# Siyou-Li/u2Tokenizer

Measured on AMD Instinct MI355X. Metric: CT volumes/sec (256^3 fp16) through u2Tokenizer fwd, higher is better.
Workload: dtype bf16; 1 GPU; BASELINE configs[2]: u2Qwen3-8B-shaped path, 256^3 volume = 8x(32,256,256) fp16, ViT-B 3D x12, SPP, 4-layer rma+diffts+dmtp tokenizer (8 heads, top_k 1024, scales {1,2,4}, 256 queries), text 1024, prompt 1024; hidden_size=4096, batch_per_gpu=1, streams_per_gpu=2, parallelism=replicas x1, tta_side_stream=off in the multi-stream run, on in the one-stream run

## Files before the change

### u2tokenizer_amd/checkpoint.py

```python
from __future__ import annotations

import os
from typing import Dict, Optional

import torch

WEIGHTS_NAME = "pytorch_model.bin"
SAFE_WEIGHTS_NAME = "model.safetensors"


def export_state_dict(model: torch.nn.Module, cpu: bool = True) -> Dict[str, torch.Tensor]:
    out = {}
    for k, v in model.state_dict().items():
        t = v.detach()
        if cpu:
            t = t.cpu()
        if not t.is_contiguous() or t.untyped_storage().nbytes() != t.numel() * t.element_size():
            t = t.clone(memory_format=torch.contiguous_format)
        out[k] = t
    return out


def save_checkpoint(model: torch.nn.Module, output_dir: str, safe_serialization: bool = False) -> str:
    os.makedirs(output_dir, exist_ok=True)
    sd = export_state_dict(model)
    if safe_serialization:
        from safetensors.torch import save_file
        path = os.path.join(output_dir, SAFE_WEIGHTS_NAME)
        save_file(sd, path, metadata={"format": "pt"})
    else:
        path = os.path.join(output_dir, WEIGHTS_NAME)
        torch.save(sd, path)
    return path


def read_checkpoint(path: str) -> Dict[str, torch.Tensor]:
    if os.path.isdir(path):
        for name in (SAFE_WEIGHTS_NAME, WEIGHTS_NAME):
            if os.path.exists(os.path.join(path, name)):
                path = os.path.join(path, name)
                break
        else:
            raise FileNotFoundError(f"no {SAFE_WEIGHTS_NAME} / {WEIGHTS_NAME} under {path}")
    if path.endswith(".safetensors"):
        from safetensors.torch import load_file
        return load_file(path)
    return torch.load(path, map_location="cpu", weights_only=True)


def load_checkpoint(model: torch.nn.Module, path_or_state_dict, strict: bool = True, prefix: Optional[str] = None,
                    offload_dead: bool = False):
    sd = path_or_state_dict if isinstance(path_or_state_dict, dict) else read_checkpoint(path_or_state_dict)
    if prefix is not None:
        sd = {k.split(prefix + ".")[1]: v for k, v in sd.items() if prefix in k}
    result = model.load_state_dict(sd, strict=strict)
    for m in model.modules():
        if hasattr(m, "pack_weights") and next(m.parameters()).is_cuda:
            m.pack_weights()
            if offload_dead:
                m.offload_dead_parameters()
    return result


def packing_report(model: torch.nn.Module) -> Dict[str, int]:
    n = packed = 0
    for m in model.modules():
        if all(hasattr(m, a) for a in ("wq", "wk", "wv")) and hasattr(m.wq, "weight"):
            n += 1
            w = [m.wq.weight, m.wk.weight, m.wv.weight]
            step = w[0].numel() * w[0].element_size()
            packed += int(all(w[i + 1].data_ptr() == w[i].data_ptr() + step for i in (0, 1)))
    return {"attention_modules": n, "qkv_packed": packed}
```

### u2tokenizer_amd/csrc/capi.hip

```cpp
#include <math.h>
#include <string.h>
#include <new>
#include "pipeline.h"

using namespace u2;

static_assert(U2TOK_OK == U2_OK && U2TOK_ERR_ARG == U2_ERR_ARG && U2TOK_ERR_LAUNCH == U2_ERR_LAUNCH &&
                  U2TOK_ERR_WORKSPACE == U2_ERR_WORKSPACE && U2TOK_ERR_DEVICE == U2_ERR_DEVICE,
              "public and internal status codes must agree");

#define BF(p) reinterpret_cast<const bf16_t*>(p)
#define BFW(p) reinterpret_cast<bf16_t*>(p)
#define ST(s) reinterpret_cast<hipStream_t>(s)

extern "C" {

int u2tok_version(void) { return 100;  }
const char* u2tok_arch(void) { return "gfx950"; }
const char* u2tok_elem(void) { return U2_ELEM_ASM; }

int u2tok_device_check(void) {
  int dev = 0;
  if (hipGetDevice(&dev) != hipSuccess) return U2_ERR_DEVICE;
  hipDeviceProp_t prop;
  if (hipGetDeviceProperties(&prop, dev) != hipSuccess) return U2_ERR_DEVICE;
  return strncmp(prop.gcnArchName, "gfx950", 6) == 0 ? U2_OK : U2_ERR_DEVICE;
}

int u2tok_ctx_create(u2tok_ctx_t* out) {
  if (!out) return U2_ERR_ARG;
  *out = reinterpret_cast<u2tok_ctx_t>(new (std::nothrow) Context());
  return *out ? U2_OK : U2_ERR_ARG;
}
int u2tok_ctx_destroy(u2tok_ctx_t c) {
  if (!c) return U2_ERR_ARG;
  Context* cx = reinterpret_cast<Context*>(c);
  if (ctx_bound() == cx) ctx_bind(nullptr);
  delete cx;
  return U2_OK;
}
int u2tok_ctx_set_current(u2tok_ctx_t c) {
  ctx_bind(reinterpret_cast<Context*>(c));
  return U2_OK;
}
u2tok_ctx_t u2tok_ctx_get_current(void) { return reinterpret_cast<u2tok_ctx_t>(ctx_bound()); }

int u2tok_set_option(const char* name, int value) {
  if (!name) return U2_ERR_ARG;
  Options& o = ctx().opt;
  struct Opt { const char* name; int Options::*field; int lo, hi; };
  static const Opt table[] = {
      {"gemm_splitk", &Options::gemm_splitk, -1, 16},   {"gemm_mubuf", &Options::gemm_mubuf, 0, 1}, {"ln_wide", &Options::ln_wide, 0, 1},   {"gemm_big", &Options::gemm_big, -1, 27},
      {"gemm_big_grid", &Options::gemm_big_grid, 1, 4096}, {"gemm_big_splitk", &Options::gemm_big_splitk, 0, 16},
      {"gemm_big_drain", &Options::gemm_big_drain, 0, 1}, {"gemm_skinny", &Options::gemm_skinny, 0, 2},
       {"kmajor_b", &Options::kmajor_b, 0, 1},            {"gemm_tail_fused", &Options::gemm_tail_fused, 0, 1},
      {"flash_mode", &Options::flash_mode, 0, 7},        {"flash_q_prescaled", &Options::flash_q_prescaled, 0, 1},
      {"vit_flash", &Options::vit_flash, 0, 1},         {"tta_overlap", &Options::tta_overlap, 0, 1},
      {"vit_vt_epilogue", &Options::vit_vt_epilogue, 0, 1},
      {"tok_flash", &Options::tok_flash, 0, 1},
      {"tok_wide", &Options::tok_wide, 0, 2},
  };
  if (!strcmp(name, "gemm_tile")) {
    if (value != 0 && value != 64 && value != 128) return U2_ERR_ARG;
    o.gemm_tile = value;
    return U2_OK;
  }
  if (!strcmp(name, "profile")) { prof_enable(value != 0); return U2_OK; }
  for (const Opt& t : table)
    if (!strcmp(name, t.name)) {
      if (value < t.lo || value > t.hi) return U2_ERR_ARG;
      if (t.field == &Options::gemm_big && value > 0 && !(value >= 20 && value <= 27 && value != 23 && value != 25)) return U2_ERR_ARG;
      if (t.field == &Options::flash_mode && value != 0 && value != 1 && value != 7) return U2_ERR_ARG;
      o.*(t.field) = value;
      return U2_OK;
    }
  return U2_ERR_ARG;
}

int u2tok_set_gemm_scratch(void* device_ptr, size_t bytes, void* stream) {
  ctx().set_scratch(reinterpret_cast<hipStream_t>(stream), device_ptr, device_ptr ? bytes : 0);
  return U2_OK;
}

int u2tok_profile_collect(double* ms, double* flops, int64_t* count, int32_t ncat) {
  if (!ms || !flops || !count || ncat <= 0 || ncat > PROF_NCAT) return U2_ERR_ARG;
  return prof_collect(ms, flops, nullptr, count, ncat);
}
int u2tok_profile_collect2(double* ms, double* flops, double* bytes, int64_t* count, int32_t ncat) {
  if (!ms || !flops || !bytes || !count || ncat <= 0 || ncat > PROF_NCAT) return U2_ERR_ARG;
  return prof_collect(ms, flops, bytes, count, ncat);
}

size_t u2tok_vit_workspace_bytes(const u2tok_vit_config* cfg) {
  if (!cfg) return 0;
  size_t peak = 0;
  if (vit_forward(*cfg, nullptr, nullptr, nullptr, nullptr, 0, true, &peak, nullptr) != U2_OK) return 0;
  return peak + 256;
}
int u2tok_vit_forward(const u2tok_vit_config* cfg, const void* const* weights, const void* volume, void* out,
                      void* workspace, size_t workspace_bytes, u2tok_stream_t stream) {
  if (!cfg || !workspace || ((uintptr_t)workspace & 255)) return U2_ERR_ARG;
  return vit_forward(*cfg, weights, volume, BFW(out), workspace, workspace_bytes, false, nullptr, ST(stream));
}

size_t u2tok_spp_workspace_bytes(const u2tok_spp_config* cfg) {
  if (!cfg) return 0;
  size_t peak = 0;
  if (spp_forward(*cfg, nullptr, nullptr, nullptr, nullptr, 0, true, &peak, nullptr) != U2_OK) return 0;
  return peak + 256;
}
int u2tok_spp_forward(const u2tok_spp_config* cfg, const void* const* weights, const void* x, void* out,
                      void* workspace, size_t workspace_bytes, u2tok_stream_t stream) {
  if (!cfg || !workspace || ((uintptr_t)workspace & 255)) return U2_ERR_ARG;
  return spp_forward(*cfg, weights, BF(x), BFW(out), workspace, workspace_bytes, false, nullptr, ST(stream));
}

size_t u2tok_tokenizer_workspace_bytes(const u2tok_tokenizer_config* cfg) {
  if (!cfg) return 0;
  size_t peak = 0;
  if (tokenizer_forward(*cfg, nullptr, nullptr, nullptr, nullptr, nullptr, nullptr, nullptr, nullptr, 0, true, &peak,
                        nullptr) != U2_OK)
    return 0;
  return peak + 256;
}
int u2tok_tokenizer_forward(const u2tok_tokenizer_config* cfg, const void* const* weights, const void* v_token,
                            const void* t_token, void* out, int64_t* topk_idx_out, void* svr_out, void* workspace,
                            size_t workspace_bytes, u2tok_stream_t stream) {
  if (!cfg || !workspace || ((uintptr_t)workspace & 255)) return U2_ERR_ARG;
  return tokenizer_forward(*cfg, weights, BF(v_token), BF(t_token), BFW(out), topk_idx_out, BFW(svr_out), nullptr, workspace,
                           workspace_bytes, false, nullptr, ST(stream));
}
int u2tok_tokenizer_forward_taps(const u2tok_tokenizer_config* cfg, const void* const* weights, const void* v_token,
                                 const void* t_token, void* out, int64_t* topk_idx_out, const u2tok_tokenizer_taps* taps,
                                 void* workspace, size_t workspace_bytes, u2tok_stream_t stream) {
  if (!cfg || !taps || !workspace || ((uintptr_t)workspace & 255)) return U2_ERR_ARG;
  return tokenizer_forward(*cfg, weights, BF(v_token), BF(t_token), BFW(out), topk_idx_out, nullptr, taps, workspace,
                           workspace_bytes, false, nullptr, ST(stream));
}

size_t u2tok_preprocess_workspace_bytes(int32_t D, int32_t H, int32_t W) { return preprocess_workspace_bytes(D, H, W); }
int u2tok_preprocess_volume(const float* vol, void* out, int32_t* info, int32_t D, int32_t H, int32_t W, int32_t target,
                            int32_t depth_pad, float lower_pct, float upper_pct, int32_t out_dtype, void* workspace,
                            size_t workspace_bytes, u2tok_stream_t stream) {
  return preprocess_volume(vol, out, info, D, H, W, target, depth_pad, lower_pct, upper_pct, out_dtype, nullptr, workspace,
                           workspace_bytes, ST(stream));
}
int u2tok_preprocess_volume_aug(const float* vol, void* out, int32_t* info, int32_t D, int32_t H, int32_t W, int32_t target,
                                int32_t depth_pad, float lower_pct, float upper_pct, int32_t out_dtype,
                                const u2tok_augment* aug, void* workspace, size_t workspace_bytes, u2tok_stream_t stream) {
  if (!aug) return U2_ERR_ARG;
  PreAugment a;
  a.rot_k = aug->rot90_k;
  for (int i = 0; i < 3; ++i) a.flip[i] = aug->flip[i];
  a.mul = 1.0f + aug->scale_factor;
  a.add = aug->shift_offset;
  return preprocess_volume(vol, out, info, D, H, W, target, depth_pad, lower_pct, upper_pct, out_dtype, &a, workspace,
                           workspace_bytes, ST(stream));
}

int u2tok_embed_splice(const void* table, const int64_t* ids, const void* feats, void* out, int32_t B, int32_t S,
                       int32_t E, int32_t nfeat, int64_t vocab, u2tok_stream_t stream) {
  return embed_splice(BF(table), ids, BF(feats), BFW(out), B, S, E, nfeat, vocab, ST(stream));
}

int u2tok_gemm_bf16(const void* A, const void* B, void* C, const void* bias, const void* R, int32_t M, int32_t N,
                    int32_t K, int64_t lda, int64_t ldb, int64_t ldc, int64_t ldr, int32_t nz, int32_t nbh,
                    int64_t sAb, int64_t sAh, int64_t sBb, int64_t sBh, int64_t sCb, int64_t sCh, int64_t sRb,
                    int64_t sRh, float alpha, int32_t flags, u2tok_stream_t stream) {
  GemmDesc g;
  g.A = BF(A); g.B = BF(B); g.C = C; g.bias = BF(bias); g.R = BF(R);
  g.M = M; g.N = N; g.K = K; g.lda = lda; g.ldb = ldb; g.ldc = ldc; g.ldr = ldr;
  g.nz = nz; g.nbh = nbh;
  g.sAb = sAb; g.sAh = sAh; g.sBb = sBb; g.sBh = sBh; g.sCb = sCb; g.sCh = sCh; g.sRb = sRb; g.sRh = sRh;
  g.alpha = alpha;
  g.flags = flags & (GEMM_BIAS_N | GEMM_BIAS_M | GEMM_GELU | GEMM_RESIDUAL | GEMM_OUT_F32 | GEMM_A_KMAJOR | GEMM_B_KMAJOR |
                     GEMM_SWIGLU);
  if (flags & GEMM_B_KTILE) {
    if ((K & 63) || nz != 1) return U2_ERR_ARG;
    g.ldb = 64;
    g.ldbk = (int64_t)N * 64;
  }
  return gemm_bf16(g, ST(stream));
}

int u2tok_layernorm_bf16(const void* x, const void* res, const void* w, const void* b, void* y, int32_t rows,
                         int32_t C, float eps, u2tok_stream_t stream) {
  return layernorm_bf16(BF(x), BF(res), BF(w), BF(b), BFW(y), 1, rows, C, 0, C, 0, C, 0, C, eps, ST(stream));
}

int u2tok_softmax_rows(const float* S, void* P, int32_t nz, int32_t rows, int32_t n, int64_t lds, int64_t ldp,
                       float scale, const void* rel_bias, int32_t H, int32_t max_len, u2tok_stream_t stream) {
  return softmax_rows(S, BFW(P), nz, rows, n, lds, ldp, (int64_t)rows * lds, (int64_t)rows * ldp, scale, BF(rel_bias), H,
                      max_len, ST(stream));
}

int u2tok_transpose_bf16(const void* in, void* out, int32_t nz, int32_t R, int32_t C, int64_t ld_in, int64_t ld_out,
                         int64_t in_zs, int64_t out_zs, int32_t perm16, u2tok_stream_t stream) {
  return transpose_bf16(BF(in), BFW(out), nz, R, C, ld_in, ld_out, in_zs, out_zs, perm16, ST(stream));
}

int u2tok_im2col_patches(const void* vol, int32_t vol_dtype, void* out, int32_t nchunk, int32_t D, int32_t H,
                         int32_t W, int32_t p1, int32_t p2, int32_t p3, u2tok_stream_t stream) {
  return im2col_patches(vol, vol_dtype, BFW(out), nchunk, D, H, W, p1, p2, p3, ST(stream));
}

int u2tok_avgpool3d_tokens(const void* x, void* y, int32_t nb, int32_t g1, int32_t g2, int32_t g3, int32_t w1,
                           int32_t w2, int32_t w3, int32_t C, u2tok_stream_t stream) {
  return avgpool3d_tokens(BF(x), BFW(y), nb, g1, g2, g3, w1, w2, w3, C, ST(stream));
}

int u2tok_score_gemv(const void* x, const void* w, const void* bias, float* scores, int32_t rows, int32_t E,
                     u2tok_stream_t stream) {
  return score_gemv(BF(x), BF(w), BF(bias), scores, rows, E, ST(stream));
}

int u2tok_topk_sorted(const float* scores, int64_t* idx, int32_t B, int32_t n, int32_t k, u2tok_stream_t stream) {
  return topk_sorted(scores, idx, B, n, k, ST(stream));
}

int u2tok_gather_rows(const void* x, const int64_t* idx, void* out, int32_t B, int32_t n, int32_t k, int32_t E,
                      u2tok_stream_t stream) {
  return gather_rows(BF(x), idx, BFW(out), B, n, k, E, ST(stream));
}

int u2tok_multiscale_pool(const void* x, void* out, int32_t B, int32_t k, int32_t E, const void* gate_w,
                          const void* gate_b, float* ws, u2tok_stream_t stream) {
  return multiscale_pool(BF(x), BFW(out), B, k, E, BF(gate_w), BF(gate_b), ws, ST(stream));
}

int u2tok_temporal_attention(const void* q, const void* k, const void* v, void* out, int32_t B, int32_t T,
                             int32_t N, int32_t H, int32_t d, int64_t ld_qkv, int64_t ld_out, float scale,
                             const void* rel_bias, int32_t max_len, u2tok_stream_t stream) {
  return temporal_attention(BF(q), BF(k), BF(v), BFW(out), B, T, N, H, d, ld_qkv, ld_out, scale, BF(rel_bias), max_len,
                            ST(stream));
}

int u2tok_flash_attention_d64(const void* q, const void* k, const void* vt, void* out, int32_t nb, int32_t S,
                              int32_t H, int64_t ld_qk, int64_t q_bs, int64_t ld_out, int64_t out_bs, int32_t S_pad,
                              float scale, const void* qx, const void* kx, const void* vx, void* outx, int64_t x_bs,
                              int64_t ox_bs, int32_t n_extra, u2tok_stream_t stream) {
  return flash_attention_d64(BF(q), BF(k), BF(vt), BFW(out), nb, S, H, ld_qk, q_bs, ld_out, out_bs, S_pad, scale,
                             BF(qx), BF(kx), BF(vx), BFW(outx), x_bs, ox_bs, n_extra, nullptr, 0, ST(stream));
}
int u2tok_flash_attention_d64_lse(const void* q, const void* k, const void* vt, void* out, int32_t nb, int32_t S,
                                  int32_t H, int64_t ld_qk, int64_t q_bs, int64_t ld_out, int64_t out_bs, int32_t S_pad,
                                  float scale, const void* qx, const void* kx, const void* vx, void* outx, int64_t x_bs,
                                  int64_t ox_bs, int32_t n_extra, float* lse, int64_t lse_ld, u2tok_stream_t stream) {
  if (!lse) return U2_ERR_ARG;
  return flash_attention_d64(BF(q), BF(k), BF(vt), BFW(out), nb, S, H, ld_qk, q_bs, ld_out, out_bs, S_pad, scale,
                             BF(qx), BF(kx), BF(vx), BFW(outx), x_bs, ox_bs, n_extra, lse, lse_ld, ST(stream));
}

size_t u2tok_tok_attention_workspace_bytes(int32_t nb, int32_t H, int32_t Sq, int32_t Skv, int32_t d) {
  return tok_attention_workspace_bytes(nb, H, Sq, Skv, d);
}
int u2tok_tok_attention(const void* q, const void* k, const void* v, void* out, int32_t nb, int32_t Sq, int32_t Skv, int32_t H,
                        int32_t d, int64_t ldq, int64_t ldk, int64_t ldv, int64_t ldo, int64_t q_bs, int64_t k_bs, int64_t v_bs,
                        int64_t o_bs, float scale, const void* rel_bias, int32_t max_len, int32_t splits, void* workspace,
                        size_t workspace_bytes, u2tok_stream_t stream) {
  return tok_attention(BF(q), BF(k), BF(v), BFW(out), nb, Sq, Skv, H, d, ldq, ldk, ldv, ldo, q_bs, k_bs, v_bs, o_bs, scale,
                       BF(rel_bias), max_len, splits, workspace, workspace_bytes, ST(stream));
}

int u2tok_attention_gqa(const void* q, const void* k, const void* v, void* out, int32_t nb, int32_t Sq, int32_t Skv, int32_t Hq,
                        int32_t Hkv, int32_t d, int64_t ldq, int64_t ldk, int64_t ldv, int64_t ldo, int64_t q_bs, int64_t k_bs,
                        int64_t v_bs, int64_t o_bs, float scale, int32_t causal, u2tok_stream_t stream) {
  return attention_ex(BF(q), BF(k), BF(v), BFW(out), nb, Sq, Skv, Hq, Hkv, d, ldq, ldk, ldv, ldo, q_bs, k_bs, v_bs, o_bs, scale,
                      nullptr, 0, causal, 1, nullptr, 0, ST(stream));
}
int u2tok_attention_gqa_split(const void* q, const void* k, const void* v, void* out, int32_t nb, int32_t Sq, int32_t Skv,
                              int32_t Hq, int32_t Hkv, int32_t d, int64_t ldq, int64_t ldk, int64_t ldv, int64_t ldo, int64_t q_bs,
                              int64_t k_bs, int64_t v_bs, int64_t o_bs, float scale, void* workspace, size_t workspace_bytes,
                              u2tok_stream_t stream) {
  return attention_ex(BF(q), BF(k), BF(v), BFW(out), nb, Sq, Skv, Hq, Hkv, d, ldq, ldk, ldv, ldo, q_bs, k_bs, v_bs, o_bs, scale,
                      nullptr, 0, 0, 0, workspace, workspace_bytes, ST(stream));
}
int u2tok_rmsnorm_bf16(const void* x, const void* w, void* y, int64_t rows, int32_t C, int64_t ldx, int64_t ldy, float eps,
                       u2tok_stream_t stream) {
  return rmsnorm_bf16(BF(x), BF(w), BFW(y), rows, C, ldx, ldy, eps, ST(stream));
}
int u2tok_qk_norm_rope(void* qkv, const void* wq, const void* wk, const void* cos, const void* sin, int32_t cos_sin_f32,
                       int64_t rows, int32_t Hq, int32_t Hkv, int32_t D, int64_t ld, int64_t cs_ld, float eps,
                       u2tok_stream_t stream) {
  return qk_norm_rope(BFW(qkv), BF(wq), BF(wk), cos, sin, cos_sin_f32, rows, Hq, Hkv, D, ld, cs_ld, eps, nullptr, nullptr, 0, 0, 0,
                      ST(stream));
}
int u2tok_qk_norm_rope_kv(void* qkv, const void* wq, const void* wk, const void* cos, const void* sin, int32_t cos_sin_f32,
                          int64_t rows, int32_t Hq, int32_t Hkv, int32_t D, int64_t ld, int64_t cs_ld, float eps,
                          void* k_cache, void* v_cache, int32_t S, int64_t kv_stride, int32_t s_off, u2tok_stream_t stream) {
  if (!k_cache || !v_cache) return U2_ERR_ARG;
  return qk_norm_rope(BFW(qkv), BF(wq), BF(wk), cos, sin, cos_sin_f32, rows, Hq, Hkv, D, ld, cs_ld, eps, BFW(k_cache),
                      BFW(v_cache), S, kv_stride, s_off, ST(stream));
}
static DecodeCfg dec_cfg(const u2tok_decode_config* c) {
  DecodeCfg d;
  d.B = c->B; d.E = c->E; d.Hq = c->Hq; d.Hkv = c->Hkv; d.D = c->D; d.I = c->I;
  d.eps = c->eps; d.qk_eps = c->qk_eps; d.scale = c->scale;
  return d;
}
static bool dec_ok(const u2tok_decode_config* c) {
  return c && c->B > 0 && c->B <= 16 && c->E > 0 && !(c->E & 31) && c->Hq > 0 && c->Hkv > 0 && c->Hq % c->Hkv == 0 &&
         (c->D == 64 || c->D == 96 || c->D == 128) && c->I > 0 && !(c->I & 31);
}
size_t u2tok_decoder_decode_workspace_bytes(const u2tok_decode_config* c, int32_t T) {
  return dec_ok(c) && T > 0 ? decoder_decode_workspace_bytes(dec_cfg(c), T) : 0;
}
int u2tok_decoder_decode_pre(const u2tok_decode_config* c, const void* x, const void* w_in_norm, const void* Wqkv, const void* bqkv,
                             const void* wq_norm, const void* wk_norm, const void* cos, const void* sin, int32_t cos_sin_f32,
                             int64_t cs_ld, void* qkv, void* k_cache, void* v_cache, int64_t kv_stride, int32_t s_off,
                             void* workspace, size_t workspace_bytes, u2tok_stream_t stream) {
  if (!dec_ok(c)) return U2_ERR_ARG;
  return decoder_decode_pre(dec_cfg(c), BF(x), BF(w_in_norm), BF(Wqkv), BF(bqkv), BF(wq_norm), BF(wk_norm), cos, sin, cos_sin_f32,
                            cs_ld, BFW(qkv), BFW(k_cache), BFW(v_cache), kv_stride, s_off, workspace, workspace_bytes, ST(stream));
}
int u2tok_decoder_decode_post(const u2tok_decode_config* c, const void* x, const void* qkv, const void* K, const void* V, int32_t T,
                              int64_t kv_stride, const void* Wo, const void* bo, const void* w_post_norm, const void* Wgu, const void* bgu,
                              const void* Wdown, const void* bdown, void* out, void* workspace, size_t workspace_bytes,
                              u2tok_stream_t stream) {
  if (!dec_ok(c)) return U2_ERR_ARG;
  return decoder_decode_post(dec_cfg(c), BF(x), BF(qkv), BF(K), BF(V), T, kv_stride, BF(Wo), BF(bo), BF(w_post_norm), BF(Wgu), BF(bgu),
                             BF(Wdown), BF(bdown), BFW(out), workspace, workspace_bytes, ST(stream));
}
int u2tok_swiglu_bf16(const void* gate_up, void* out, int64_t rows, int32_t I, int64_t ld_in, int64_t ld_out,
                      u2tok_stream_t stream) {
  return swiglu_bf16(BF(gate_up), BFW(out), rows, I, ld_in, ld_out, ST(stream));
}

int u2tok_rope_apply(void* x, int64_t n_outer, int32_t S, int32_t n_inner, int32_t H, int32_t d, int64_t ld,
                     int32_t max_len, int32_t inverse, u2tok_stream_t stream) {
  return rope_apply(BFW(x), n_outer, S, n_inner, H, d, ld, max_len, inverse, ST(stream));
}

int u2tok_gelu_fwd(const void* z, void* y, int64_t n, u2tok_stream_t stream) { return gelu_fwd(BF(z), BFW(y), n, ST(stream)); }
int u2tok_gelu_bwd(const void* z, const void* dy, void* dz, int64_t n, u2tok_stream_t stream) {
  return gelu_bwd(BF(z), BF(dy), BFW(dz), n, ST(stream));
}
size_t u2tok_colsum_workspace_bytes(int32_t rows, int32_t C) { return colsum_workspace_bytes(rows, C); }
int u2tok_colsum_bf16(const void* x, const void* y, float* out, void* out_bf16, int32_t rows, int32_t C, int64_t ldx,
                      int64_t ldy, void* workspace, int32_t accumulate, u2tok_stream_t stream) {
  return colsum_bf16(BF(x), BF(y), out, BFW(out_bf16), rows, C, ldx, ldy, reinterpret_cast<float*>(workspace), accumulate,
                     ST(stream));
}
size_t u2tok_layernorm_bwd_workspace_bytes(int32_t rows, int32_t C) { return layernorm_bwd_workspace_bytes(rows, C); }
int u2tok_layernorm_bwd(const void* x, const void* res, const void* w, const void* dy, void* dv, float* dw, float* db,
                        int32_t rows, int32_t C, float eps, void* workspace, int32_t accumulate, u2tok_stream_t stream) {
  return layernorm_bwd(BF(x), BF(res), BF(w), BF(dy), BFW(dv), dw, db, rows, C, eps, reinterpret_cast<float*>(workspace),
                       accumulate, ST(stream));
}
int u2tok_softmax_bwd(const void* P, const float* dP, void* dS, int64_t nrows, int32_t n, int64_t ldp, int64_t lddp,
                      u2tok_stream_t stream) {
  return softmax_bwd(BF(P), dP, BFW(dS), nrows, n, ldp, lddp, ST(stream));
}
int u2tok_relbias_grad(const void* dS, float* dtable, int32_t nz, int32_t S, int32_t H, int64_t ldp, int32_t max_len,
                       u2tok_stream_t stream) {
  return relbias_grad(BF(dS), dtable, nz, S, H, ldp, max_len, ST(stream));
}
int u2tok_rowdot_bf16(const void* a, const void* b, float* out, int64_t rows, int32_t C, int64_t lda, int64_t ldb,
                      u2tok_stream_t stream) {
  return rowdot_bf16(BF(a), BF(b), out, rows, C, lda, ldb, ST(stream));
}
int u2tok_ce_lse_update(const void* Z, int64_t ldz, int32_t rows, int32_t Vs, int64_t v0, const int64_t* labels, float* m, float* l,
                        float* zt, u2tok_stream_t stream) {
  return ce_lse_update(BF(Z), ldz, rows, Vs, v0, labels, m, l, zt, ST(stream));
}
int u2tok_ce_grad_inplace(void* Z, int64_t ldz, int32_t rows, int32_t Vs, int64_t v0, const int64_t* labels, const float* lse,
                          const float* coef, u2tok_stream_t stream) {
  return ce_grad_inplace(BFW(Z), ldz, rows, Vs, v0, labels, lse, coef, ST(stream));
}
int u2tok_adamw_step(float* master, float* exp_avg, float* exp_avg_sq, const void* grad, const uint8_t* group, void* out_bf16,
                     int64_t n, const float* lr, const float* weight_decay, int32_t ngroups, float beta1, float beta2, float eps,
                     int32_t step, float grad_scale, const float* grad_coef, u2tok_stream_t stream) {
  if (!lr || !weight_decay || ngroups <= 0 || ngroups > 8 || step <= 0 || (ngroups > 1 && !group)) return U2_ERR_ARG;
  AdamWArgs a;
  for (int i = 0; i < 8; ++i) { a.lr[i] = lr[i < ngroups ? i : 0]; a.wd[i] = weight_decay[i < ngroups ? i : 0]; }
  a.b1 = beta1; a.b2 = beta2; a.eps = eps;
  a.inv_c1 = (float)(1.0 / (1.0 - pow((double)beta1, step)));
  a.inv_sqrt_c2 = (float)(1.0 / sqrt(1.0 - pow((double)beta2, step)));
  a.gscale = grad_scale; a.gcoef = grad_coef;
  return adamw_step(master, exp_avg, exp_avg_sq, BF(grad), group, BFW(out_bf16), n, a, ST(stream));
}
size_t u2tok_flash_attention_d64_bwd_workspace_bytes(int32_t nb, int32_t S, int32_t H) {
  return flash_attention_d64_bwd_workspace_bytes(nb, S, H);
}
int32_t u2tok_flash_attention_d64_bwd(const void* q, const void* k, const void* v, int64_t ld_qkv, int64_t bs_qkv,
                                      const void* out, const void* d_out, int64_t ld_o, int64_t bs_o, void* dq, void* dk,
                                      void* dv, int64_t ld_d, int64_t bs_d, int32_t nb, int32_t S, int32_t H, float scale,
                                      const float* lse, int64_t lse_ld, void* workspace, size_t workspace_bytes,
                                      u2tok_stream_t stream) {
  return flash_attention_d64_bwd(BF(q), BF(k), BF(v), ld_qkv, bs_qkv, BF(out), BF(d_out), ld_o, bs_o, BFW(dq), BFW(dk), BFW(dv),
                                 ld_d, bs_d, nb, S, H, scale, lse, lse_ld, workspace, workspace_bytes, ST(stream));
}

int u2tok_attention_gqa_ex(const void* q, const void* k, const void* v, void* out, int32_t nb, int32_t Sq, int32_t Skv,
                           int32_t Hq, int32_t Hkv, int32_t d, int64_t ldq, int64_t ldk, int64_t ldv, int64_t ldo, int64_t q_bs,
                           int64_t k_bs, int64_t v_bs, int64_t o_bs, float scale, int32_t causal, const int32_t* kv_len,
                           float* lse, int64_t lse_ld, u2tok_stream_t stream) {
  return attention_gqa_ex(BF(q), BF(k), BF(v), BFW(out), nb, Sq, Skv, Hq, Hkv, d, ldq, ldk, ldv, ldo, q_bs, k_bs, v_bs, o_bs,
                          scale, causal, kv_len, lse, lse_ld, ST(stream));
}
size_t u2tok_attention_gqa_bwd_workspace_bytes(int32_t nb, int32_t S, int32_t Hq) {
  return attention_gqa_bwd_workspace_bytes(nb, S, Hq);
}
int u2tok_attention_gqa_bwd(const void* q, const void* k, const void* v, int64_t ld_qkv, int64_t bs_qkv, const void* out,
                            const void* d_out, int64_t ld_o, int64_t bs_o, void* dq, void* dk, void* dv, int64_t ld_d, int64_t bs_d,
                            int32_t nb, int32_t S, int32_t Hq, int32_t Hkv, int32_t d, float scale, const int32_t* kv_len,
                            const float* lse, int64_t lse_ld, void* workspace, size_t workspace_bytes, u2tok_stream_t stream) {
  return attention_gqa_bwd(BF(q), BF(k), BF(v), ld_qkv, bs_qkv, BF(out), BF(d_out), ld_o, bs_o, BFW(dq), BFW(dk), BFW(dv), ld_d,
                           bs_d, nb, S, Hq, Hkv, d, scale, kv_len, lse, lse_ld, workspace, workspace_bytes, ST(stream));
}
size_t u2tok_rmsnorm_bwd_workspace_bytes(int32_t rows, int32_t C) { return rmsnorm_bwd_workspace_bytes(rows, C); }
int u2tok_rmsnorm_bwd(const void* x, const void* w, const void* dy, const void* dres, void* dx, float* dw, int32_t rows, int32_t C,
                      float eps, void* workspace, size_t workspace_bytes, int32_t accumulate, u2tok_stream_t stream) {
  return rmsnorm_bwd(BF(x), BF(w), BF(dy), BF(dres), BFW(dx), dw, rows, C, eps, reinterpret_cast<float*>(workspace),
                     workspace_bytes, accumulate, ST(stream));
}
size_t u2tok_qk_norm_rope_bwd_workspace_bytes(int64_t rows, int32_t D) { return qk_norm_rope_bwd_workspace_bytes(rows, D); }
int u2tok_qk_norm_rope_bwd(void* dqkv, const void* pre, const void* wq, const void* wk, const void* cos, const void* sin,
                           int32_t cos_sin_f32, int64_t rows, int32_t Hq, int32_t Hkv, int32_t D, int64_t ld, int64_t ld_pre,
                           int64_t cs_ld, float eps, float* dwq, float* dwk, void* workspace, size_t workspace_bytes,
                           int32_t accumulate, u2tok_stream_t stream) {
  return qk_norm_rope_bwd(BFW(dqkv), BF(pre), BF(wq), BF(wk), cos, sin, cos_sin_f32, rows, Hq, Hkv, D, ld, ld_pre, cs_ld, eps, dwq,
                          dwk, reinterpret_cast<float*>(workspace), workspace_bytes, accumulate, ST(stream));
}
int u2tok_swiglu_bwd(const void* gu, const void* dact, void* dgu, int64_t rows, int32_t I, int64_t ld_gu, int64_t ld_da,
                     int64_t ld_dgu, u2tok_stream_t stream) {
  return swiglu_bwd(BF(gu), BF(dact), BFW(dgu), rows, I, ld_gu, ld_da, ld_dgu, ST(stream));
}

}
```

### u2tokenizer_amd/csrc/ctx.h

```cpp
#pragma once
#include <mutex>
#include <vector>
#include "common.h"

namespace u2 {

struct Options {
  int ln_wide = 1;
  int gemm_tile = 0;
  int gemm_mubuf = 1;
  int gemm_splitk = 0;
  int gemm_big = 0;
  int gemm_big_grid = 256;
  int gemm_big_splitk = 0;
  int gemm_big_drain = 1;
  int gemm_skinny = 2;
  int gemm_tail_fused = 1;
  int kmajor_b = 1;
  int flash_mode = 0;
  int flash_q_prescaled = 0;
  int vit_flash = 1;
  int vit_vt_epilogue = 1;
  int tok_flash = 1;
  int tok_wide = 2;
  int tta_overlap = 1;
  int profile = 0;
};

struct SideStream {
  hipStream_t owner = nullptr;
  hipStream_t s = nullptr;
  hipEvent_t fork = nullptr;
  hipEvent_t done[16] = {};
};

struct Scratch {
  hipStream_t st;
  void* p;
  size_t bytes;
};

struct ProfRec {
  hipEvent_t a, b;
  int cat;
  double flops, bytes;
};

struct Context {
  Options opt;
  std::mutex mu;
  std::vector<SideStream*> sides;
  std::vector<Scratch> scratch;
  std::vector<ProfRec> recs;
  std::vector<hipEvent_t> ev_pool;
  size_t ev_used = 0;

  SideStream* side_for(hipStream_t owner);
  void set_scratch(hipStream_t st, void* p, size_t bytes);
  Scratch scratch_of(hipStream_t st);
  void release();
  ~Context() { release(); }
};

Context& ctx();
void ctx_bind(Context* c);
Context* ctx_bound();
inline const Options& opts() { return ctx().opt; }

}
```

### u2tokenizer_amd/csrc/ctx.hip

```cpp
#include "kernels.h"

namespace u2 {

namespace {
Context g_default_ctx;
thread_local Context* tl_ctx = nullptr;
}

Context& ctx() { return tl_ctx ? *tl_ctx : g_default_ctx; }
void ctx_bind(Context* c) { tl_ctx = c; }
Context* ctx_bound() { return tl_ctx; }

SideStream* Context::side_for(hipStream_t owner) {
  std::lock_guard<std::mutex> lk(mu);
  for (SideStream* s : sides)
    if (s->owner == owner) return s;
  SideStream* s = new SideStream();
  s->owner = owner;
  bool ok = hipStreamCreateWithFlags(&s->s, hipStreamNonBlocking) == hipSuccess &&
            hipEventCreateWithFlags(&s->fork, hipEventDisableTiming) == hipSuccess;
  for (auto& e : s->done) ok = ok && hipEventCreateWithFlags(&e, hipEventDisableTiming) == hipSuccess;
  if (!ok) {
    (void)hipGetLastError();
    delete s;
    return nullptr;
  }
  sides.push_back(s);
  return s;
}

void Context::set_scratch(hipStream_t st, void* p, size_t bytes) {
  std::lock_guard<std::mutex> lk(mu);
  for (auto& s : scratch)
    if (s.st == st) { s.p = p; s.bytes = bytes; return; }
  scratch.push_back({st, p, bytes});
}

Scratch Context::scratch_of(hipStream_t st) {
  std::lock_guard<std::mutex> lk(mu);
  for (auto& s : scratch)
    if (s.st == st) return s;
  return {st, nullptr, 0};
}

void Context::release() {
  std::lock_guard<std::mutex> lk(mu);
  for (SideStream* s : sides) {
    (void)hipStreamDestroy(s->s);
    (void)hipEventDestroy(s->fork);
    for (auto& e : s->done) (void)hipEventDestroy(e);
    delete s;
  }
  sides.clear();
  for (hipEvent_t e : ev_pool) (void)hipEventDestroy(e);
  ev_pool.clear();
  recs.clear();
  ev_used = 0;
}

void prof_enable(bool on) {
  Context& c = ctx();
  std::lock_guard<std::mutex> lk(c.mu);
  c.opt.profile = on ? 1 : 0;
  c.recs.clear();
  c.ev_used = 0;
}
bool prof_enabled() { return opts().profile != 0; }

ProfScope::ProfScope(int cat, double flops, hipStream_t st, double bytes) : idx_(-1), st_(st), c_(nullptr) {
  Context& c = ctx();
  if (!c.opt.profile) return;
  std::lock_guard<std::mutex> lk(c.mu);
  auto get_event = [&]() -> hipEvent_t {
    if (c.ev_used == c.ev_pool.size()) {
      hipEvent_t e;
      if (hipEventCreate(&e) != hipSuccess) return nullptr;
      c.ev_pool.push_back(e);
    }
    return c.ev_pool[c.ev_used++];
  };
  ProfRec r{get_event(), get_event(), cat, flops, bytes};
  if (!r.a || !r.b) return;
  (void)hipEventRecord(r.a, st);
  c.recs.push_back(r);
  idx_ = (int)c.recs.size() - 1;
  c_ = &c;
}
ProfScope::~ProfScope() {
  if (idx_ < 0) return;
  std::lock_guard<std::mutex> lk(c_->mu);
  if ((size_t)idx_ < c_->recs.size()) (void)hipEventRecord(c_->recs[idx_].b, st_);
}

int prof_collect(double* ms, double* flops, double* bytes, int64_t* count, int ncat) {
  Context& c = ctx();
  std::lock_guard<std::mutex> lk(c.mu);
  for (int i = 0; i < ncat; ++i) { ms[i] = 0; flops[i] = 0; count[i] = 0; if (bytes) bytes[i] = 0; }
  int rc = U2_OK;
  for (auto& r : c.recs) {
    float t = 0.f;
    if (hipEventSynchronize(r.b) != hipSuccess || hipEventElapsedTime(&t, r.a, r.b) != hipSuccess) { rc = U2_ERR_LAUNCH; break; }
    if (r.cat >= 0 && r.cat < ncat) {
      ms[r.cat] += t; flops[r.cat] += r.flops; count[r.cat] += 1;
      if (bytes) bytes[r.cat] += r.bytes;
    }
  }
  c.recs.clear();
  c.ev_used = 0;
  return rc;
}

}
```

### u2tokenizer_amd/csrc/pipeline.hip

```cpp
#include "pipeline.h"

namespace u2 {

namespace {

struct Arena {
  char* base;
  size_t cap;
  size_t off = 0, peak = 0;
  bool dry;
  Arena(void* b, size_t c, bool d) : base((char*)b), cap(c), dry(d) {}
  template <typename T>
  T* get(size_t count) {
    const size_t a = (off + 255) & ~(size_t)255;
    off = a + count * sizeof(T);
    if (off > peak) peak = off;
    if (dry) return reinterpret_cast<T*>((uintptr_t)0x1000 + a);
    return (off <= cap) ? reinterpret_cast<T*>(base + a) : nullptr;
  }
  bool ok() const { return dry || peak <= cap; }
};

struct ScratchScope {
  Context& cx;
  hipStream_t st;
  Scratch prev;
  bool on;
  ScratchScope(Context& c, hipStream_t s, void* p, size_t bytes, bool enable) : cx(c), st(s), prev{s, nullptr, 0}, on(enable) {
    if (!on) return;
    prev = cx.scratch_of(st);
    cx.set_scratch(st, p, bytes);
  }
  ~ScratchScope() { if (on) cx.set_scratch(st, prev.p, prev.bytes); }
};

#define U2_RUN(expr)                  \
  do {                                \
    if (!dry) {                       \
      const int e_ = (expr);          \
      if (e_ != U2_OK) return e_;     \
    }                                 \
  } while (0)
#define U2_CHECK_WS(ar) \
  do {                  \
    if (!(ar).ok()) return U2_ERR_WORKSPACE; \
  } while (0)

inline int64_t round_up(int64_t x, int64_t m) { return (x + m - 1) / m * m; }

static GemmDesc linear_desc(const bf16_t* x, int64_t ldx, const bf16_t* w, const bf16_t* b, bf16_t* y, int64_t ldy, int64_t rows,
                            int in, int out, int extra_flags, const bf16_t* R, int64_t ldr, int nsplit, float alpha_lo) {
  GemmDesc g;
  g.A = x; g.B = w; g.C = y; g.bias = b; g.R = R;
  g.M = (int)rows; g.N = out; g.K = in;
  g.lda = ldx; g.ldb = in; g.ldc = ldy; g.ldr = ldr;
  g.flags = (b ? GEMM_BIAS_N : 0) | extra_flags | (R ? GEMM_RESIDUAL : 0);
  g.nsplit = nsplit; g.alpha_lo = alpha_lo;
  return g;
}

int linear(const bf16_t* x, int64_t ldx, const bf16_t* w, const bf16_t* b, bf16_t* y, int64_t ldy, int64_t rows,
           int in, int out, int extra_flags, const bf16_t* R, int64_t ldr, hipStream_t st, int nsplit = 0,
           float alpha_lo = 1.f) {
  return gemm_bf16(linear_desc(x, ldx, w, b, y, ldy, rows, in, out, extra_flags, R, ldr, nsplit, alpha_lo), st);
}

struct AttnCore {
  const bf16_t *q, *k, *v;
  int64_t ldq, ldk, ldv, q_bs, k_bs, v_bs;
  bf16_t* out;
  int64_t ldo, o_bs;
  int nb, Sq, Skv, H, d;
  float scale;
  const bf16_t* rel_bias;
  int max_len;
  bool unfused = false;
};

int attention_core(Arena& ar, const AttnCore& a, bool dry, hipStream_t st) {
  if (!a.unfused && (dry || opts().tok_flash)) {
    const size_t mark = ar.off;
    const size_t wsb = tok_attention_workspace_bytes(a.nb, a.H, a.Sq, a.Skv, a.d);
    char* tws = wsb ? ar.get<char>(wsb) : nullptr;
    U2_CHECK_WS(ar);
    if (!dry && tok_attention_supported(a.q, a.k, a.v, a.out, a.Sq, a.Skv, a.d, a.ldq, a.ldk, a.ldv, a.ldo, a.q_bs, a.k_bs,
                                        a.v_bs, a.o_bs, a.rel_bias, a.max_len)) {
      const int e = tok_attention(a.q, a.k, a.v, a.out, a.nb, a.Sq, a.Skv, a.H, a.d, a.ldq, a.ldk, a.ldv, a.ldo, a.q_bs,
                                  a.k_bs, a.v_bs, a.o_bs, a.scale, a.rel_bias, a.max_len, 0, tws, wsb, st);
      ar.off = mark;
      return e;
    }
    ar.off = mark;
  }
  const size_t mark = ar.off;
  const int64_t ldS = round_up(a.Skv, 8), ldp = ldS;
  const int64_t nz = (int64_t)a.nb * a.H;
  if (nz > 65535) return U2_ERR_ARG;
  float* S = ar.get<float>((size_t)nz * a.Sq * ldS);
  bf16_t* P = ar.get<bf16_t>((size_t)nz * a.Sq * ldp);
  const bool v_in_place = opts().kmajor_b && !(a.Skv & 7) && !(a.d & 7) && !(a.ldv & 7) && !(a.v_bs & 7) && !((uintptr_t)a.v & 15);
  bf16_t* Vt = v_in_place ? nullptr : ar.get<bf16_t>((size_t)a.nb * a.H * a.d * ldp);
  U2_CHECK_WS(ar);
  {
    GemmDesc g;
    g.A = a.q; g.B = a.k; g.C = S;
    g.M = a.Sq; g.N = a.Skv; g.K = a.d;
    g.lda = a.ldq; g.ldb = a.ldk; g.ldc = ldS;
    g.nz = (int)nz; g.nbh = a.H;
    g.sAb = a.q_bs; g.sAh = a.d; g.sBb = a.k_bs; g.sBh = a.d;
    g.sCb = (int64_t)a.H * a.Sq * ldS; g.sCh = (int64_t)a.Sq * ldS;
    g.flags = GEMM_OUT_F32;
    U2_RUN(gemm_bf16(g, st));
  }
  U2_RUN(softmax_rows(S, P, (int)nz, a.Sq, a.Skv, ldS, ldp, (int64_t)a.Sq * ldS, (int64_t)a.Sq * ldp, a.scale,
                      a.rel_bias, a.H, a.max_len, st));
  {
    GemmDesc g;
    g.A = P; g.C = a.out;
    g.M = a.Sq; g.N = a.d;
    g.lda = ldp; g.ldc = a.ldo;
    g.nz = (int)nz; g.nbh = a.H;
    g.sAb = (int64_t)a.H * a.Sq * ldp; g.sAh = (int64_t)a.Sq * ldp;
    g.sCb = a.o_bs; g.sCh = a.d;
    if (v_in_place) {
      g.B = a.v; g.K = a.Skv; g.ldb = a.ldv;
      g.sBb = a.v_bs; g.sBh = a.d;
      g.flags = GEMM_B_KMAJOR;
    } else {
      U2_RUN(transpose_bf16(a.v, Vt, a.nb, a.Skv, a.H * a.d, a.ldv, ldp, a.v_bs, (int64_t)a.H * a.d * ldp, 0, st));
      g.B = Vt; g.K = (int)ldp; g.ldb = ldp;
      g.sBb = (int64_t)a.H * a.d * ldp; g.sBh = (int64_t)a.d * ldp;
    }
    U2_RUN(gemm_bf16(g, st));
  }
  ar.off = mark;
  return U2_OK;
}

int chunk_axis_attention(Arena& ar, const bf16_t* qkv, bf16_t* out, int Bx, int Tx, int Nx, int H, int d, float scale,
                         const bf16_t* rel_bias, int max_len, bool dry, hipStream_t st) {
  const int E = H * d;
  if (Tx <= 16 && (d == 64 || d == 128 || d == 256 || d == 512)) {
    U2_RUN(temporal_attention(qkv, qkv + E, qkv + 2 * E, out, Bx, Tx, Nx, H, d, 3 * E, E, scale, rel_bias, max_len, st));
    return U2_OK;
  }
  for (int b = 0; b < Bx; ++b) {
    const bf16_t* base = qkv + (int64_t)b * Tx * Nx * 3 * E;
    AttnCore a{base, base + E, base + 2 * E, (int64_t)Nx * 3 * E, (int64_t)Nx * 3 * E, (int64_t)Nx * 3 * E, 3 * E, 3 * E,
               3 * E, out + (int64_t)b * Tx * Nx * E, (int64_t)Nx * E, E, Nx, Tx, Tx, H, d, scale, rel_bias, max_len};
    const int e = attention_core(ar, a, dry, st);
    if (e != U2_OK) return e;
  }
  return U2_OK;
}

}

int vit_forward(const VitConfig& c, const void* const* W, const void* volume, bf16_t* out, void* ws, size_t ws_bytes,
                bool dry, size_t* peak, hipStream_t st) {
  if (c.nchunk <= 0 || c.depth < 0 || c.heads <= 0 || c.hidden != c.heads * 64) return U2_ERR_ARG;
  for (int i = 0; i < 3; ++i)
    if (c.img[i] <= 0 || c.patch[i] <= 0 || c.img[i] % c.patch[i]) return U2_ERR_ARG;
  if (!dry && (!W || !volume || !out)) return U2_ERR_ARG;
  const int nh = c.img[0] / c.patch[0], nw = c.img[1] / c.patch[1], nd = c.img[2] / c.patch[2];
  const int ntok = nh * nw * nd, S = ntok + 1, Hd = c.hidden, Kp = c.patch[0] * c.patch[1] * c.patch[2];
  const int nc = c.nchunk;
  const int64_t prow = (int64_t)nc * ntok;
  const int64_t rows = prow + nc;
  const int S_pad = (int)round_up(ntok, 64);
  auto w = [&](int i) { return dry ? nullptr : reinterpret_cast<const bf16_t*>(W[i]); };

  ScratchScope scratch_scope(ctx(), st, nullptr, 0, !dry);
  Arena ar(ws, ws_bytes, dry);
  bf16_t* x = ar.get<bf16_t>((size_t)rows * Hd);
  bf16_t* xn = ar.get<bf16_t>((size_t)rows * Hd);
  bf16_t* qkv = ar.get<bf16_t>((size_t)rows * 3 * Hd);
  bf16_t* att = ar.get<bf16_t>((size_t)rows * Hd);
  bf16_t* vt = ar.get<bf16_t>((size_t)nc * Hd * S_pad);
  const size_t big = std::max((size_t)nc * ntok * Kp, (size_t)rows * c.mlp_dim);
  bf16_t* h1 = ar.get<bf16_t>(big);
  bf16_t* patches = h1;
  U2_CHECK_WS(ar);

  U2_RUN(im2col_patches(volume, c.vol_dtype, patches, nc, c.img[0], c.img[1], c.img[2], c.patch[0], c.patch[1],
                        c.patch[2], st));
  U2_RUN(fill_rows(w(3), x + prow * Hd, nc, Hd, Hd, st));
  {
    GemmDesc g;
    g.A = patches; g.B = w(1); g.C = x; g.bias = w(2); g.R = w(0);
    g.M = ntok; g.N = Hd; g.K = Kp;
    g.lda = Kp; g.ldb = Kp; g.ldc = Hd; g.ldr = Hd;
    g.nz = nc; g.nbh = 1;
    g.sAb = (int64_t)ntok * Kp; g.sCb = (int64_t)ntok * Hd;
    g.flags = GEMM_BIAS_N | GEMM_RESIDUAL;
    U2_RUN(gemm_bf16(g, st));
  }
  const float scale = 1.0f / sqrtf(64.0f);
  for (int l = 0; l < c.depth; ++l) {
    const int b0 = 4 + 11 * l;
    U2_RUN(layernorm_bf16(x, nullptr, w(b0 + 0), w(b0 + 1), xn, 1, (int)rows, Hd, 0, Hd, 0, 0, 0, Hd, c.ln_eps, st));
    const bool q_pre = opts().vit_flash && ntok >= 512 && (opts().flash_mode == 0 || opts().flash_mode == 7);
    GemmDesc gq = linear_desc(xn, Hd, w(b0 + 2), nullptr, qkv, 3 * Hd, rows, Hd, 3 * Hd, 0, nullptr, 0, q_pre ? Hd : 0,
                              scale * 1.44269504088896340736f);
    const bool vt_fused = opts().vit_flash && opts().vit_vt_epilogue && S_pad == ntok && gemm_vt_supported(gq, 2 * Hd, ntok);
    if (vt_fused) {
      gq.vt = vt; gq.vt_n0 = 2 * Hd; gq.vt_rows = ntok; gq.vt_ld = S_pad; gq.vt_bs = (int64_t)Hd * S_pad;
    }
    U2_RUN(gemm_bf16(gq, st));
    if (opts().vit_flash) {
      if (!vt_fused)
        U2_RUN(transpose_bf16(qkv + 2 * Hd, vt, nc, ntok, Hd, 3 * Hd, S_pad, (int64_t)ntok * 3 * Hd, (int64_t)Hd * S_pad, 1, st));
      const bf16_t* xq = qkv + prow * 3 * Hd;
      U2_RUN(flash_attention_d64(qkv, qkv + Hd, vt, att, nc, ntok, c.heads, 3 * Hd, (int64_t)ntok * 3 * Hd, Hd,
                                 (int64_t)ntok * Hd, S_pad, scale, xq, xq + Hd, xq + 2 * Hd, att + prow * Hd, 3 * Hd, Hd,
                                 1, nullptr, 0, st, q_pre ? 1 : 0));
    } else {
      const size_t mark = ar.off;
      bf16_t* qc = ar.get<bf16_t>((size_t)rows * 3 * Hd);
      bf16_t* ac = ar.get<bf16_t>((size_t)rows * Hd);
      U2_CHECK_WS(ar);
      const size_t rb = (size_t)3 * Hd * sizeof(bf16_t), ob = (size_t)Hd * sizeof(bf16_t);
      if (!dry) {
        const hipError_t e1 = hipMemcpy2DAsync(qc + 3 * Hd, (size_t)S * rb, qkv, (size_t)ntok * rb, (size_t)ntok * rb, nc,
                                               hipMemcpyDeviceToDevice, st);
        const hipError_t e2 = hipMemcpy2DAsync(qc, (size_t)S * rb, qkv + prow * 3 * Hd, rb, rb, nc,
                                               hipMemcpyDeviceToDevice, st);
        if (e1 != hipSuccess || e2 != hipSuccess) return U2_ERR_LAUNCH;
      }
      {
        AttnCore a{qc, qc + Hd, qc + 2 * Hd, 3 * Hd, 3 * Hd, 3 * Hd, (int64_t)S * 3 * Hd, (int64_t)S * 3 * Hd,
                   (int64_t)S * 3 * Hd, ac, Hd, (int64_t)S * Hd, nc, S, S, c.heads, 64, scale, nullptr, 0, true};
        const int e = attention_core(ar, a, dry, st);
        if (e != U2_OK) return e;
      }
      if (!dry) {
        const hipError_t e1 = hipMemcpy2DAsync(att, (size_t)ntok * ob, ac + Hd, (size_t)S * ob, (size_t)ntok * ob, nc,
                                               hipMemcpyDeviceToDevice, st);
        const hipError_t e2 = hipMemcpy2DAsync(att + prow * Hd, ob, ac, (size_t)S * ob, ob, nc, hipMemcpyDeviceToDevice, st);
        if (e1 != hipSuccess || e2 != hipSuccess) return U2_ERR_LAUNCH;
      }
      ar.off = mark;
    }
    U2_RUN(linear(att, Hd, w(b0 + 3), w(b0 + 4), x, Hd, rows, Hd, Hd, 0, x, Hd, st));
    U2_RUN(layernorm_bf16(x, nullptr, w(b0 + 5), w(b0 + 6), xn, 1, (int)rows, Hd, 0, Hd, 0, 0, 0, Hd, c.ln_eps, st));
    U2_RUN(linear(xn, Hd, w(b0 + 7), w(b0 + 8), h1, c.mlp_dim, rows, Hd, c.mlp_dim, GEMM_GELU, nullptr, 0, st));
    U2_RUN(linear(h1, c.mlp_dim, w(b0 + 9), w(b0 + 10), x, Hd, rows, c.mlp_dim, Hd, 0, x, Hd, st));
  }
  const int nwt = 4 + 11 * c.depth;
  if (c.keep_cls) {
    U2_RUN(layernorm_bf16(x, nullptr, w(nwt), w(nwt + 1), out + Hd, nc, ntok, Hd, (int64_t)ntok * Hd, Hd, 0, 0,
                          (int64_t)S * Hd, Hd, c.ln_eps, st));
    U2_RUN(layernorm_bf16(x + prow * Hd, nullptr, w(nwt), w(nwt + 1), out, nc, 1, Hd, Hd, Hd, 0, 0, (int64_t)S * Hd, Hd,
                          c.ln_eps, st));
  } else {
    U2_RUN(layernorm_bf16(x, nullptr, w(nwt), w(nwt + 1), out, 1, (int)prow, Hd, 0, Hd, 0, 0, 0, Hd, c.ln_eps, st));
  }
  if (peak) *peak = ar.peak;
  U2_CHECK_WS(ar);
  return U2_OK;
}

int spp_forward(const SppConfig& c, const void* const* W, const bf16_t* x, bf16_t* out, void* ws, size_t ws_bytes,
                bool dry, size_t* peak, hipStream_t st) {
  if (c.nchunk <= 0 || c.pooling_size <= 0 || c.layer_num <= 0 || c.in_dim <= 0 || c.out_dim <= 0) return U2_ERR_ARG;
  if (!dry && (!W || !x || !out)) return U2_ERR_ARG;
  const int ps = c.pooling_size;
  int g1 = c.grid[0], g2 = c.grid[1], g3 = c.grid[2], w1 = ps, w2 = ps, w3 = ps;
  if (c.pooling_type == 1) { g3 = g1 * g2 * g3; g1 = g2 = 1; w1 = w2 = 1; w3 = ps * ps * ps; }
  else if (c.pooling_type != 0) return U2_ERR_ARG;
  if (g1 < w1 || g2 < w2 || g3 < w3) return U2_ERR_ARG;
  const int np = (g1 / w1) * (g2 / w2) * (g3 / w3);
  const int64_t rows = (int64_t)c.nchunk * np;
  auto w = [&](int i) { return dry ? nullptr : reinterpret_cast<const bf16_t*>(W[i]); };
  ScratchScope scratch_scope(ctx(), st, nullptr, 0, !dry);
  Arena ar(ws, ws_bytes, dry);
  bf16_t* pooled = ar.get<bf16_t>((size_t)rows * c.in_dim);
  bf16_t* ha = ar.get<bf16_t>((size_t)rows * c.out_dim);
  bf16_t* hb = ar.get<bf16_t>((size_t)rows * c.out_dim);
  U2_CHECK_WS(ar);
  U2_RUN(avgpool3d_tokens(x, pooled, c.nchunk, g1, g2, g3, w1, w2, w3, c.in_dim, st));
  const bf16_t* cur = pooled;
  int cur_dim = c.in_dim;
  for (int l = 0; l < c.layer_num; ++l) {
    const bool last = (l == c.layer_num - 1);
    bf16_t* dst = last ? out : ((l & 1) ? hb : ha);
    const int fl = (!last && c.layer_type == 0) ? GEMM_GELU : 0;
    U2_RUN(linear(cur, cur_dim, w(2 * l), w(2 * l + 1), dst, c.out_dim, rows, cur_dim, c.out_dim, fl, nullptr, 0, st));
    cur = dst;
    cur_dim = c.out_dim;
  }
  if (peak) *peak = ar.peak;
  return U2_OK;
}

namespace {
struct Att {
  const bf16_t *wq, *bq, *wk, *bk, *wv, *bv, *wd, *bd, *rb;
};
inline bool kv_packed(const Att& a, int E) {
  return a.wk && a.bk && a.wv == a.wk + (size_t)E * E && a.bv == a.bk + E;
}
inline bool qkv_packed(const Att& a, int E) {
  return a.wq && a.bq && a.wk == a.wq + (size_t)E * E && a.bk == a.bq + E && kv_packed(a, E);
}
int qkv_proj(const bf16_t* x, const Att& a, bf16_t* out, int64_t rows, int E, bool dry, hipStream_t st) {
  if (!dry && qkv_packed(a, E)) {
    U2_RUN(linear(x, E, a.wq, a.bq, out, 3 * E, rows, E, 3 * E, 0, nullptr, 0, st));
    return U2_OK;
  }
  U2_RUN(linear(x, E, a.wq, a.bq, out, 3 * E, rows, E, E, 0, nullptr, 0, st));
  U2_RUN(linear(x, E, a.wk, a.bk, out + E, 3 * E, rows, E, E, 0, nullptr, 0, st));
  U2_RUN(linear(x, E, a.wv, a.bv, out + 2 * E, 3 * E, rows, E, E, 0, nullptr, 0, st));
  return U2_OK;
}
}

int tokenizer_forward(const TokConfig& c, const void* const* W, const bf16_t* v_token, const bf16_t* t_token,
                      bf16_t* out, int64_t* topk_idx_out, bf16_t* svr_out, const TokTaps* taps, void* ws, size_t ws_bytes,
                      bool dry, size_t* peak, hipStream_t st) {
  if (c.B <= 0 || c.T <= 0 || c.N <= 0 || c.E <= 0 || c.Lt <= 0 || c.num_heads <= 0 || c.num_layers < 0) return U2_ERR_ARG;
  if (c.E % c.num_heads || (c.E / c.num_heads) % 8 || c.top_k <= 0 || c.num_query <= 0) return U2_ERR_ARG;
  if (c.attn_type < 0 || c.attn_type > 2) return U2_ERR_ARG;
  if (!dry && (!W || !v_token || !t_token || !out)) return U2_ERR_ARG;
  const int B = c.B, T = c.T, N = c.N, E = c.E, H = c.num_heads, d = E / H, L = c.num_layers, Q = c.num_query;
  const int TN = T * N, k = c.top_k;
  if (!c.enable_diffts && k > TN) return U2_ERR_ARG;
  if (N > c.max_seq_len || T > c.max_seq_len || Q > c.max_seq_len) return U2_ERR_ARG;
  const float scale = 1.0f / sqrtf((float)d);
  auto wp = [&](int i) { return dry ? nullptr : reinterpret_cast<const bf16_t*>(W[i]); };
  auto att_at = [&](int i) {
    Att a{wp(i), wp(i + 1), wp(i + 2), wp(i + 3), wp(i + 4), wp(i + 5), wp(i + 6), wp(i + 7), wp(i + 8)};
    if (c.attn_type != 0) a.rb = nullptr;
    return a;
  };
  const int i_sel = 1 + 18 * L, i_gate = i_sel + 2, i_tta = i_gate + 2, i_lin = i_tta + 33 * L;

  Arena ar(ws, ws_bytes, dry);
  const size_t kSplitK = std::max<size_t>(24u << 20, (size_t)16 * B * c.num_query * 3 * E);
  char* skw = ar.get<char>(kSplitK);
  U2_CHECK_WS(ar);
  Context& cx = ctx();
  ScratchScope scratch_scope(cx, st, skw, kSplitK, !dry);
  const int64_t rows = (int64_t)B * TN;
  bf16_t* xa = ar.get<bf16_t>((size_t)rows * E);
  bf16_t* xb = ar.get<bf16_t>((size_t)rows * E);
  bf16_t* qkv = ar.get<bf16_t>((size_t)rows * 3 * E);
  bf16_t* ctx = ar.get<bf16_t>((size_t)rows * E);
  U2_CHECK_WS(ar);

  const bf16_t* x = v_token;
  for (int l = 0; l < L; ++l) {
    const Att sp = att_at(1 + 18 * l), tp = att_at(1 + 18 * l + 9);
    if (taps && !dry && taps->svr_in && taps->svr_in[l]) x = reinterpret_cast<const bf16_t*>(taps->svr_in[l]);
    bf16_t* y = (x == xa) ? xb : xa;
    { const int e = qkv_proj(x, sp, qkv, rows, E, dry, st); if (e != U2_OK) return e; }
    if (c.attn_type == 1) {
      U2_RUN(rope_apply(qkv, (int64_t)B * T, N, 1, H, d, 3 * E, c.max_seq_len, 0, st));
      U2_RUN(rope_apply(qkv + E, (int64_t)B * T, N, 1, H, d, 3 * E, c.max_seq_len, 0, st));
    }
    if (c.attn_type == 2) {
      const int e = chunk_axis_attention(ar, qkv, ctx, 1, B * T, N, H, d, scale, nullptr, c.max_seq_len, dry, st);
      if (e != U2_OK) return e;
    } else {
      AttnCore a{qkv, qkv + E, qkv + 2 * E, 3 * E, 3 * E, 3 * E, (int64_t)N * 3 * E, (int64_t)N * 3 * E,
                 (int64_t)N * 3 * E, ctx, E, (int64_t)N * E, B * T, N, N, H, d, scale, sp.rb, c.max_seq_len};
      const int e = attention_core(ar, a, dry, st);
      if (e != U2_OK) return e;
    }
    U2_RUN(linear(ctx, E, sp.wd, sp.bd, y, E, rows, E, E, 0, nullptr, 0, st));
    bf16_t* y2 = (y == xa) ? xb : xa;
    { const int e = qkv_proj(y, tp, qkv, rows, E, dry, st); if (e != U2_OK) return e; }
    if (c.attn_type == 1) {
      U2_RUN(rope_apply(qkv, B, T, N, H, d, 3 * E, c.max_seq_len, 0, st));
      U2_RUN(rope_apply(qkv + E, B, T, N, H, d, 3 * E, c.max_seq_len, 0, st));
    }
    if (c.attn_type == 2 && B == 1) {
      AttnCore a{qkv, qkv + E, qkv + 2 * E, 3 * E, 3 * E, 3 * E, (int64_t)N * 3 * E, (int64_t)N * 3 * E,
                 (int64_t)N * 3 * E, ctx, E, (int64_t)N * E, T, N, N, H, d, scale, nullptr, 0};
      const int e = attention_core(ar, a, dry, st);
      if (e != U2_OK) return e;
    } else if (c.attn_type == 2) {
      const size_t mark = ar.off;
      bf16_t* g = ar.get<bf16_t>((size_t)rows * 3 * E);
      bf16_t* gc = ar.get<bf16_t>((size_t)rows * E);
      U2_CHECK_WS(ar);
      if (!dry)
        for (int b = 0; b < B; ++b)
          if (hipMemcpy2DAsync(g + (size_t)b * N * 3 * E, (size_t)B * N * 3 * E * 2, qkv + (size_t)b * T * N * 3 * E,
                               (size_t)N * 3 * E * 2, (size_t)N * 3 * E * 2, T, hipMemcpyDeviceToDevice, st) != hipSuccess)
            return U2_ERR_LAUNCH;
      const int64_t S2 = (int64_t)B * N;
      AttnCore a{g, g + E, g + 2 * E, 3 * E, 3 * E, 3 * E, S2 * 3 * E, S2 * 3 * E, S2 * 3 * E, gc, E, S2 * E,
                 T, (int)S2, (int)S2, H, d, scale, nullptr, 0};
      const int e = attention_core(ar, a, dry, st);
      if (e != U2_OK) return e;
      if (!dry)
        for (int b = 0; b < B; ++b)
          if (hipMemcpy2DAsync(ctx + (size_t)b * T * N * E, (size_t)N * E * 2, gc + (size_t)b * N * E, (size_t)B * N * E * 2,
                               (size_t)N * E * 2, T, hipMemcpyDeviceToDevice, st) != hipSuccess)
            return U2_ERR_LAUNCH;
      ar.off = mark;
    } else {
      const int e = chunk_axis_attention(ar, qkv, ctx, B, T, N, H, d, scale, tp.rb, c.max_seq_len, dry, st);
      if (e != U2_OK) return e;
    }
    U2_RUN(linear(ctx, E, tp.wd, tp.bd, y2, E, rows, E, E, 0, nullptr, 0, st));
    x = y2;
    if (taps && !dry && taps->svr_out && taps->svr_out[l] &&
        hipMemcpyAsync(taps->svr_out[l], x, (size_t)rows * E * sizeof(bf16_t), hipMemcpyDeviceToDevice, st) != hipSuccess)
      return U2_ERR_LAUNCH;
  }

  if (svr_out && !dry) {
    if (hipMemcpyAsync(svr_out, x, (size_t)rows * E * sizeof(bf16_t), hipMemcpyDeviceToDevice, st) != hipSuccess)
      return U2_ERR_LAUNCH;
  }

  bf16_t* sel = ar.get<bf16_t>((size_t)B * k * E);
  U2_CHECK_WS(ar);
  if (c.enable_diffts) {
    const size_t mark = ar.off;
    const int64_t ldS = round_up(TN, 8);
    float* scT = ar.get<float>((size_t)B * k * ldS);
    bf16_t* P = ar.get<bf16_t>((size_t)B * k * ldS);
    const bool x_in_place = opts().kmajor_b && !(TN & 7);
    bf16_t* Xt = x_in_place ? nullptr : ar.get<bf16_t>((size_t)B * E * ldS);
    U2_CHECK_WS(ar);
    {
      GemmDesc g;
      g.A = wp(i_sel); g.B = x; g.C = scT; g.bias = wp(i_sel + 1);
      g.M = k; g.N = TN; g.K = E; g.lda = E; g.ldb = E; g.ldc = ldS;
      g.nz = B; g.sBb = (int64_t)TN * E; g.sCb = (int64_t)k * ldS;
      g.flags = GEMM_BIAS_M | GEMM_OUT_F32;
      U2_RUN(gemm_bf16(g, st));
    }
    U2_RUN(softmax_rows(scT, P, B, k, TN, ldS, ldS, (int64_t)k * ldS, (int64_t)k * ldS, 1.0f / c.diffts_tau, nullptr, 1,
                        0, st));
    {
      GemmDesc g;
      g.A = P; g.C = sel;
      g.M = k; g.N = E; g.lda = ldS; g.ldc = E;
      g.nz = B; g.sAb = (int64_t)k * ldS; g.sCb = (int64_t)k * E;
      if (x_in_place) {
        g.B = x; g.K = TN; g.ldb = E; g.sBb = (int64_t)TN * E;
        g.flags = GEMM_B_KMAJOR;
      } else {
        U2_RUN(transpose_bf16(x, Xt, B, TN, E, E, ldS, (int64_t)TN * E, (int64_t)E * ldS, 0, st));
        g.B = Xt; g.K = (int)ldS; g.ldb = ldS; g.sBb = (int64_t)E * ldS;
      }
      U2_RUN(gemm_bf16(g, st));
    }
    ar.off = mark;
  } else {
    const size_t mark = ar.off;
    float* scores = ar.get<float>((size_t)rows);
    int64_t* idx = topk_idx_out ? topk_idx_out : ar.get<int64_t>((size_t)B * k);
    U2_CHECK_WS(ar);
    U2_RUN(score_gemv(x, wp(i_sel), wp(i_sel + 1), scores, (int)rows, E, st));
    U2_RUN(topk_sorted(scores, idx, B, TN, k, st));
    U2_RUN(gather_rows(x, idx, sel, B, TN, k, E, st));
    ar.off = mark;
  }

  const bf16_t* V = sel;
  int Lv = k;
  if (c.use_multi_scale) {
    Lv = k + k / 2 + k / 4;
    bf16_t* pooled = ar.get<bf16_t>((size_t)B * Lv * E);
    float* gws = ar.get<float>((size_t)B * 3 * 16 * cdiv(E, 256));
    U2_CHECK_WS(ar);
    U2_RUN(multiscale_pool(sel, pooled, B, k, E, c.enable_dmtp ? wp(i_gate) : nullptr,
                           c.enable_dmtp ? wp(i_gate + 1) : nullptr, gws, st));
    V = pooled;
  }
  if (taps && !dry) {
    if (taps->visual_out &&
        hipMemcpyAsync(taps->visual_out, V, (size_t)B * Lv * E * sizeof(bf16_t), hipMemcpyDeviceToDevice, st) != hipSuccess)
      return U2_ERR_LAUNCH;
    if (taps->visual_in) V = reinterpret_cast<const bf16_t*>(taps->visual_in);
  }

  const int64_t qrows = (int64_t)B * Q;
  bf16_t* qa = ar.get<bf16_t>((size_t)qrows * E);
  bf16_t* qb = ar.get<bf16_t>((size_t)qrows * E);
  bf16_t* qc = ar.get<bf16_t>((size_t)qrows * E);
  bf16_t* qproj = ar.get<bf16_t>((size_t)qrows * 3 * E);
  bf16_t* qctx = ar.get<bf16_t>((size_t)qrows * E);
  bf16_t* qo = ar.get<bf16_t>((size_t)qrows * E);
  SideStream* side = (!dry && opts().tta_overlap && L > 0 && L <= 7) ? cx.side_for(st) : nullptr;
  const bool overlap = dry ? (L > 0 && L <= 7) : side != nullptr;
  const int Lmax = Lv > c.Lt ? Lv : c.Lt;
  bf16_t* kv_inline = overlap ? nullptr : ar.get<bf16_t>((size_t)B * Lmax * 2 * E);
  bf16_t* kv_v[8] = {};
  bf16_t* kv_t[8] = {};
  if (overlap)
    for (int l = 0; l < L; ++l) {
      kv_v[l] = ar.get<bf16_t>((size_t)B * Lv * 2 * E);
      kv_t[l] = ar.get<bf16_t>((size_t)B * c.Lt * 2 * E);
    }
  bf16_t* k_lin = ar.get<bf16_t>((size_t)B * Lv * E);
  U2_CHECK_WS(ar);
  auto kv_proj = [&](const Att& a, const bf16_t* src, int Ls, bf16_t* kv, hipStream_t s_) -> int {
    if (!dry && kv_packed(a, E)) {
      U2_RUN(linear(src, E, a.wk, a.bk, kv, 2 * E, (int64_t)B * Ls, E, 2 * E, 0, nullptr, 0, s_));
    } else {
      U2_RUN(linear(src, E, a.wk, a.bk, kv, 2 * E, (int64_t)B * Ls, E, E, 0, nullptr, 0, s_));
      U2_RUN(linear(src, E, a.wv, a.bv, kv + E, 2 * E, (int64_t)B * Ls, E, E, 0, nullptr, 0, s_));
    }
    return U2_OK;
  };
  if (overlap && !dry) {
    if (hipEventRecord(side->fork, st) != hipSuccess || hipStreamWaitEvent(side->s, side->fork, 0) != hipSuccess)
      return U2_ERR_LAUNCH;
    for (int l = 0; l < L; ++l) {
      const int base = i_tta + 33 * l;
      Att va = att_at(base + 9), ta = att_at(base + 18);
      { const int e = kv_proj(va, V, Lv, kv_v[l], side->s); if (e != U2_OK) return e; }
      if (hipEventRecord(side->done[2 * l], side->s) != hipSuccess) return U2_ERR_LAUNCH;
      { const int e = kv_proj(ta, t_token, c.Lt, kv_t[l], side->s); if (e != U2_OK) return e; }
      if (hipEventRecord(side->done[2 * l + 1], side->s) != hipSuccess) return U2_ERR_LAUNCH;
    }
    const Att la = att_at(i_lin);
    U2_RUN(linear(V, E, la.wk, la.bk, k_lin, E, (int64_t)B * Lv, E, E, 0, nullptr, 0, side->s));
    if (hipEventRecord(side->done[2 * L], side->s) != hipSuccess) return U2_ERR_LAUNCH;
  }
  U2_RUN(fill_rows(wp(0), qa, B, (int64_t)Q * E, (int64_t)Q * E, st));
  bf16_t* qcur = qa;
  auto cross = [&](const Att& a, const bf16_t* src, int Ls, const bf16_t* qin, bf16_t* dst, bf16_t* kv,
                   int kv_ready) -> int {
    U2_RUN(linear(qin, E, a.wq, a.bq, qproj, E, qrows, E, E, 0, nullptr, 0, st));
    if (kv_ready < 0) {
      const int e = kv_proj(a, src, Ls, kv, st);
      if (e != U2_OK) return e;
    } else if (!dry) {
      if (hipStreamWaitEvent(st, side->done[kv_ready], 0) != hipSuccess) return U2_ERR_LAUNCH;
    }
    AttnCore ac{qproj, kv, kv + E, E, 2 * E, 2 * E, (int64_t)Q * E, (int64_t)Ls * 2 * E, (int64_t)Ls * 2 * E,
                qctx, E, (int64_t)Q * E, B, Q, Ls, H, d, scale, nullptr, 0};
    const int e = attention_core(ar, ac, dry, st);
    if (e != U2_OK) return e;
    U2_RUN(linear(qctx, E, a.wd, a.bd, dst, E, qrows, E, E, 0, nullptr, 0, st));
    return U2_OK;
  };
  for (int l = 0; l < L; ++l) {
    const int base = i_tta + 33 * l;
    const Att sa = att_at(base);
    Att va = att_at(base + 9), ta = att_at(base + 18);
    va.rb = ta.rb = nullptr;
    const bf16_t *ns_w = wp(base + 27), *ns_b = wp(base + 28), *nv_w = wp(base + 29), *nv_b = wp(base + 30),
                 *nt_w = wp(base + 31), *nt_b = wp(base + 32);
    if (taps && !dry && taps->tta_in && taps->tta_in[l]) qcur = (bf16_t*)taps->tta_in[l];
    bf16_t* s1 = (qcur == qa) ? qb : qa;
    bf16_t* s2 = qc;
    if (c.attn_type == 2 && B == 1) {
      U2_RUN(linear(qcur, E, sa.wv, sa.bv, qctx, E, qrows, E, E, 0, nullptr, 0, st));
    } else if (c.attn_type == 2) {
      { const int e = qkv_proj(qcur, sa, qproj, qrows, E, dry, st); if (e != U2_OK) return e; }
      const int e = chunk_axis_attention(ar, qproj, qctx, 1, B, Q, H, d, scale, nullptr, c.max_seq_len, dry, st);
      if (e != U2_OK) return e;
    } else {
      { const int e = qkv_proj(qcur, sa, qproj, qrows, E, dry, st); if (e != U2_OK) return e; }
      if (c.attn_type == 1) {
        U2_RUN(rope_apply(qproj, B, Q, 1, H, d, 3 * E, c.max_seq_len, 0, st));
        U2_RUN(rope_apply(qproj + E, B, Q, 1, H, d, 3 * E, c.max_seq_len, 0, st));
      }
      AttnCore ac{qproj, qproj + E, qproj + 2 * E, 3 * E, 3 * E, 3 * E, (int64_t)Q * 3 * E, (int64_t)Q * 3 * E,
                  (int64_t)Q * 3 * E, qctx, E, (int64_t)Q * E, B, Q, Q, H, d, scale, sa.rb, c.max_seq_len};
      const int e = attention_core(ar, ac, dry, st);
      if (e != U2_OK) return e;
    }
    U2_RUN(linear(qctx, E, sa.wd, sa.bd, qo, E, qrows, E, E, 0, nullptr, 0, st));
    U2_RUN(layernorm_bf16(qcur, qo, ns_w, ns_b, s1, 1, (int)qrows, E, 0, E, 0, E, 0, E, c.ln_eps, st));
    { const int e = cross(va, V, Lv, s1, qo, overlap ? kv_v[l] : kv_inline, overlap ? 2 * l : -1); if (e != U2_OK) return e; }
    U2_RUN(layernorm_bf16(s1, qo, nv_w, nv_b, s2, 1, (int)qrows, E, 0, E, 0, E, 0, E, c.ln_eps, st));
    { const int e = cross(ta, t_token, c.Lt, s2, qo, overlap ? kv_t[l] : kv_inline, overlap ? 2 * l + 1 : -1); if (e != U2_OK) return e; }
    U2_RUN(layernorm_bf16(s2, qo, nt_w, nt_b, s1, 1, (int)qrows, E, 0, E, 0, E, 0, E, c.ln_eps, st));
    qcur = s1;
    if (taps && !dry && taps->tta_out && taps->tta_out[l] &&
        hipMemcpyAsync(taps->tta_out[l], qcur, (size_t)qrows * E * sizeof(bf16_t), hipMemcpyDeviceToDevice, st) != hipSuccess)
      return U2_ERR_LAUNCH;
  }
  {
    const Att la = att_at(i_lin);
    U2_RUN(linear(qcur, E, la.wq, la.bq, qproj, E, qrows, E, E, 0, nullptr, 0, st));
    if (!overlap) {
      U2_RUN(linear(V, E, la.wk, la.bk, k_lin, E, (int64_t)B * Lv, E, E, 0, nullptr, 0, st));
    } else if (!dry) {
      if (hipStreamWaitEvent(st, side->done[2 * L], 0) != hipSuccess) return U2_ERR_LAUNCH;
    }
    AttnCore ac{qproj, k_lin, V, E, E, E, (int64_t)Q * E, (int64_t)Lv * E, (int64_t)Lv * E,
                out, E, (int64_t)Q * E, B, Q, Lv, H, d, scale, nullptr, 0};
    const int e = attention_core(ar, ac, dry, st);
    if (e != U2_OK) return e;
  }
  if (peak) *peak = ar.peak;
  U2_CHECK_WS(ar);
  return U2_OK;
}

}
```

### u2tokenizer_amd/csrc/tokattn.hip

```cpp
#include "kernels.h"
#if U2_ELEM_IS_F16
#include "build_f16/tokattn_pv_asm.inc"
#else
#include "tokattn_pv_asm.inc"
#endif

namespace u2 {

struct TokAttnArgs {
  const bf16_t *q, *k, *v;
  bf16_t* out;
  int64_t ldq, ldk, ldv, ldo, q_bs, k_bs, v_bs, o_bs;
  int nb, H, Sq, Skv, nqb;
  int ns, tps;
  float scale_log2e;
  const bf16_t* rel_bias;
  int max_len;
  float* opart;
  float* ml;
  int kv_group;
  int causal;
  const int* kv_len;
  float* lse;
  int64_t lse_ld;
};

constexpr float TOKATTN_RESCALE_THR = 8.0f;
constexpr int TOKATTN_BIAS_SLOTS = 640;

template <int SEG>
__device__ __forceinline__ int tv_rot(int k) {
  if constexpr (SEG == 16) return 2 * (k & 3) + 8 * ((k >> 2) & 1);
  else return 2 * ((k >> 1) & 1) + 4 * ((k >> 2) & 1);
}

__device__ __forceinline__ int t96_pos(int row, int L) { return L ^ ((row >> 1) & 2); }

typedef short ta_v4s_t __attribute__((ext_vector_type(4)));

template <int DH, bool EX = false>
__global__ __launch_bounds__(256, DH >= 512 ? 1 : 2) void tok_attn_kernel(const TokAttnArgs a) {
  constexpr int BK = DH <= 128 ? 64 : 32;
  constexpr int NKB = BK / 16;
  constexpr int NPF = BK / 32;
  constexpr int CPR = DH / 8;
  constexpr int ROWB = DH * 2;
  constexpr int TILE = BK * ROWB;
  constexpr int SEG = CPR >= 16 ? 16 : 8;
  constexpr int NP = BK * CPR / 256;
  constexpr int KS = DH / 32;
  constexpr int DB = DH / 16;
  static_assert(NP >= 1 && BK * CPR % 256 == 0, "tile");
  extern __shared__ __attribute__((aligned(16))) char lds[];
  float* const sbias = reinterpret_cast<float*>(lds + 4 * TILE);

  const int tid = threadIdx.x;
  const int lane = tid & 63;
  const int w = __builtin_amdgcn_readfirstlane(tid >> 6);
  const int l15 = lane & 15, g = lane >> 4;

  int bid;
  {
    const int nwg = gridDim.x, qn = nwg >> 3, rn = nwg & 7;
    const int xcd = blockIdx.x & 7, idx = blockIdx.x >> 3;
    bid = (xcd < rn ? xcd * (qn + 1) : rn * (qn + 1) + (xcd - rn) * qn) + idx;
  }
  const int qblk = a.causal ? a.nqb - 1 - bid % a.nqb : bid % a.nqb;
  const int sp = (bid / a.nqb) % a.ns;
  const int bh = bid / (a.nqb * a.ns);
  const int b = bh / a.H, h = bh - b * a.H;
  const int q0 = qblk * 64;
  const int Sq = a.Sq, Skv = a.Skv;
  const int ntile_all = (Skv + BK - 1) / BK;
  const int c_off = Skv - Sq;
  int kt1_ = min(ntile_all, sp * a.tps + a.tps);
  if (a.causal) kt1_ = min(kt1_, (q0 + 63 + c_off) / BK + 1);
  int kvl = Skv;
  if constexpr (EX) {
    if (a.kv_len) {
      kvl = max(1, min(a.kv_len[b], Skv));
      kt1_ = min(kt1_, (kvl + BK - 1) / BK);
    }
  }
  const int kt0 = sp * a.tps, kt1 = kt1_;
  const int kbeg = kt0 * BK;

  const int hkv = h / a.kv_group;
  const bf16_t* kb_ = a.k + (int64_t)b * a.k_bs + hkv * DH;
  const bf16_t* vb_ = a.v + (int64_t)b * a.v_bs + hkv * DH;

  const int qrow = q0 + 16 * w + l15;
  bf16x8 qf[KS];
  {
    const bf16_t* qp = a.q + (int64_t)b * a.q_bs + (int64_t)min(qrow, Sq - 1) * a.ldq + h * DH + g * 8;
#pragma unroll
    for (int ks = 0; ks < KS; ++ks) qf[ks] = *reinterpret_cast<const bf16x8*>(qp + ks * 32);
  }
  const bool has_bias = a.rel_bias != nullptr;
  if (has_bias) {
    const int tmin = kbeg - (q0 + 63) + a.max_len - 1;
    const int nslot = (kt1 - kt0) * BK + 63;
    for (int t = tid; t < nslot; t += 256) {
      const int row = tmin + t;
      float v = 0.f;
      if (row >= 0 && row < 2 * a.max_len - 1) v = bf16_to_f32(a.rel_bias[(int64_t)row * a.H + h]) * 1.44269504088896340736f;
      sbias[t] = v;
    }
  }

  auto dma_k = [&](int kt, int stage) {
    char* const sK = lds + stage * 2 * TILE;
#pragma unroll
    for (int i = 0; i < NP; ++i) {
      const int c = i * 256 + w * 64 + lane, row = CPR >= 64 ? (i * 256 + w * 64) / CPR : c / CPR, cp = c % CPR;
      const int src_chunk = DH == 96 ? t96_pos(row, cp) : cp ^ (row & (SEG - 1));
      const bf16_t* src = kb_ + (int64_t)min(kt * BK + row, Skv - 1) * a.ldk + src_chunk * 8;
      __builtin_amdgcn_global_load_lds((const __attribute__((address_space(1))) void*)src,
                                       (__attribute__((address_space(3))) void*)(sK + (i * 256 + w * 64) * 16), 16, 0, 0);
    }
  };
  auto dma_v = [&](int kt, int stage) {
    char* const sV = lds + stage * 2 * TILE + TILE;
#pragma unroll
    for (int i = 0; i < NP; ++i) {
      const int c = i * 256 + w * 64 + lane, row = CPR >= 64 ? (i * 256 + w * 64) / CPR : c / CPR, cp = c % CPR;
      const int src_chunk = DH == 96 ? t96_pos(row, cp) : (cp & ~(SEG - 1)) | (((cp & (SEG - 1)) - tv_rot<SEG>(row)) & (SEG - 1));
      const bf16_t* src = vb_ + (int64_t)min(kt * BK + row, Skv - 1) * a.ldv + src_chunk * 8;
      __builtin_amdgcn_global_load_lds((const __attribute__((address_space(1))) void*)src,
                                       (__attribute__((address_space(3))) void*)(sV + (i * 256 + w * 64) * 16), 16, 0, 0);
    }
  };

  const int k_row_off = l15 * ROWB;
  const int k_swz = DH == 96 ? (l15 >> 1) & 2 : l15 & (SEG - 1);
  const int v_row = 4 * g + (l15 >> 2);
  const int v_rot = tv_rot<SEG>(v_row);
  const int v_base_off = v_row * ROWB + (l15 & 1) * 8;
  const int v_cc = (l15 & 3) >> 1;

  f32x4 o[DB];
#pragma unroll
  for (int db = 0; db < DB; ++db) o[db] = f32x4{0.f, 0.f, 0.f, 0.f};
  float m_run = -INFINITY, l_run = 0.f;
  const float c_scale = a.scale_log2e;
  const int bias_q = q0 + 63 - qrow;

  typedef __attribute__((address_space(3))) ta_v4s_t* lds_v4;

  if (kt0 < kt1) {
    dma_k(kt0, 0);
    dma_v(kt0, 0);
  }
  for (int kt = kt0; kt < kt1; ++kt) {
    const int stage = (kt - kt0) & 1;
    const char* const tK = lds + stage * 2 * TILE;
    const char* const tV = tK + TILE;
    asm volatile("s_waitcnt vmcnt(0)" ::: "memory");
    __syncthreads();
    if (kt + 1 < kt1) dma_k(kt + 1, stage ^ 1);
    f32x4 sc[NKB];
    {
      constexpr int NQK = NKB * KS, PD = NQK < 8 ? NQK : 8;
      f32x4 acc[NKB][2];
#pragma unroll
      for (int kb = 0; kb < NKB; ++kb) acc[kb][0] = acc[kb][1] = f32x4{0.f, 0.f, 0.f, 0.f};
      bf16x8 kf[NQK];
      __builtin_amdgcn_sched_barrier(0);
#pragma unroll
      for (int i = 0; i < NQK; ++i)
        kf[i] = *reinterpret_cast<const bf16x8*>(tK + (i % NKB) * 16 * ROWB + k_row_off + ((((i / NKB) * 4 + g) ^ k_swz) << 4));
#pragma unroll
      for (int i = 0; i < NQK; ++i)
        acc[i % NKB][(i / NKB) & 1] =
            mfma16(kf[i], qf[i / NKB], acc[i % NKB][(i / NKB) & 1]);
      __builtin_amdgcn_sched_group_barrier(0x100, PD, 0);
#pragma unroll
      for (int i = 0; i < NQK; ++i) {
        __builtin_amdgcn_sched_group_barrier(0x008, 1, 0);
        if (i + PD < NQK) __builtin_amdgcn_sched_group_barrier(0x100, 1, 0);
      }
      __builtin_amdgcn_sched_barrier(0);
#pragma unroll
      for (int kb = 0; kb < NKB; ++kb) sc[kb] = KS > 1 ? acc[kb][0] + acc[kb][1] : acc[kb][0];
    }
    constexpr int NX = 4 * NKB;
    float x[NX];
    if (has_bias) {
      float bb[NX];
#pragma unroll
      for (int i = 0; i < NX; ++i) bb[i] = sbias[(kt * BK - kbeg) + (i >> 2) * 16 + 4 * g + (i & 3) + bias_q];
#pragma unroll
      for (int i = 0; i < NX; ++i) x[i] = __builtin_fmaf(sc[i >> 2][i & 3], c_scale, bb[i]);
    } else {
#pragma unroll
      for (int i = 0; i < NX; ++i) x[i] = sc[i >> 2][i & 3];
    }
    if (kt == ntile_all - 1 && (Skv & (BK - 1))) {
#pragma unroll
      for (int i = 0; i < NX; ++i)
        if (kt * BK + (i >> 2) * 16 + 4 * g + (i & 3) >= Skv) x[i] = -INFINITY;
    }
    if (a.causal && kt * BK + BK - 1 > q0 + 16 * w + c_off) {
#pragma unroll
      for (int i = 0; i < NX; ++i)
        if (kt * BK + (i >> 2) * 16 + 4 * g + (i & 3) > qrow + c_off) x[i] = -INFINITY;
    }
    if constexpr (EX) {
      if (kt * BK + BK > kvl) {
#pragma unroll
        for (int i = 0; i < NX; ++i)
          if (kt * BK + (i >> 2) * 16 + 4 * g + (i & 3) >= kvl) x[i] = -INFINITY;
      }
    }
    float mt = x[0];
#pragma unroll
    for (int i = 1; i < NX; ++i) mt = fmaxf(mt, x[i]);
    mt = fmaxf(mt, __shfl_xor(mt, 16, 64));
    mt = fmaxf(mt, __shfl_xor(mt, 32, 64));
    const float xs = has_bias ? 1.0f : c_scale;
    mt *= xs;
    if (__any(mt > m_run + TOKATTN_RESCALE_THR)) {
      const float m_new = fmaxf(m_run, mt);
      const float alpha = __builtin_amdgcn_exp2f(m_run - m_new);
      m_run = m_new;
      l_run *= alpha;
#pragma unroll
      for (int db = 0; db < DB; ++db) {
        o[db][0] *= alpha; o[db][1] *= alpha; o[db][2] *= alpha; o[db][3] *= alpha;
      }
    }
    float ps = 0.f;
#pragma unroll
    for (int i = 0; i < NX; ++i) {
      x[i] = __builtin_amdgcn_exp2f(__builtin_fmaf(x[i], xs, -m_run));
      ps += x[i];
    }
    l_run += ps;
    union { bf16x8 v; uint32_t u[4]; } pf[NPF];
#pragma unroll
    for (int j = 0; j < NPF; ++j) {
      pf[j].u[0] = pack2_bf16(x[8 * j + 0], x[8 * j + 1]);
      pf[j].u[1] = pack2_bf16(x[8 * j + 2], x[8 * j + 3]);
      pf[j].u[2] = pack2_bf16(x[8 * j + 4], x[8 * j + 5]);
      pf[j].u[3] = pack2_bf16(x[8 * j + 6], x[8 * j + 7]);
    }

    if (kt + 1 < kt1) dma_v(kt + 1, stage ^ 1);
    {
      constexpr int NPV = NPF * DB, PD = NPV < 6 ? NPV : 6;
      bf16x8 vf[NPV];
      __builtin_amdgcn_sched_barrier(0);
#pragma unroll
      for (int i = 0; i < NPV; ++i) {
        const int cc = 2 * (i % DB) + v_cc;
        const int cp = DH == 96 ? t96_pos(v_row, cc) : (cc & ~(SEG - 1)) | (((cc & (SEG - 1)) + v_rot) & (SEG - 1));
        const char* p = tV + (i / DB) * 32 * ROWB + v_base_off + cp * 16;
        const ta_v4s_t lo = __builtin_amdgcn_ds_read_tr16_b64_v4i16((lds_v4)p);
        const ta_v4s_t hi = __builtin_amdgcn_ds_read_tr16_b64_v4i16((lds_v4)(p + 16 * ROWB));
        vf[i] = bf16x8{lo[0], lo[1], lo[2], lo[3], hi[0], hi[1], hi[2], hi[3]};
      }
#pragma unroll
      for (int i = 0; i < NPV; ++i)
        o[i % DB] = mfma16(vf[i], pf[i / DB].v, o[i % DB]);
      __builtin_amdgcn_sched_group_barrier(0x100, 2 * PD, 0);
#pragma unroll
      for (int i = 0; i < NPV; ++i) {
        __builtin_amdgcn_sched_group_barrier(0x008, 1, 0);
        if (i + PD < NPV) __builtin_amdgcn_sched_group_barrier(0x100, 2, 0);
      }
      __builtin_amdgcn_sched_barrier(0);
    }
  }

  float l_tot = l_run + __shfl_xor(l_run, 16, 64);
  l_tot += __shfl_xor(l_tot, 32, 64);
  if (qrow >= Sq) return;
  if constexpr (EX) {
    if (a.lse && g == 0) a.lse[((int64_t)b * a.H + h) * a.lse_ld + qrow] = m_run + __builtin_log2f(l_tot);
  }
  if (a.ns == 1) {
    const float inv = 1.f / l_tot;
    bf16_t* op = a.out + (int64_t)b * a.o_bs + (int64_t)qrow * a.ldo + h * DH + 4 * g;
#pragma unroll
    for (int db = 0; db < DB; ++db)
      *reinterpret_cast<uint2*>(op + db * 16) =
          uint2{pack2_bf16(o[db][0] * inv, o[db][1] * inv), pack2_bf16(o[db][2] * inv, o[db][3] * inv)};
  } else {
    const int E = a.H * DH;
    float* pp = a.opart + (((int64_t)sp * a.nb + b) * Sq + qrow) * E + h * DH + 4 * g;
#pragma unroll
    for (int db = 0; db < DB; ++db) *reinterpret_cast<float4*>(pp + db * 16) = float4{o[db][0], o[db][1], o[db][2], o[db][3]};
    if (g == 0) {
      float* mp = a.ml + ((((int64_t)sp * a.nb + b) * a.H + h) * Sq + qrow) * 2;
      mp[0] = m_run;
      mp[1] = l_tot;
    }
  }
}

__device__ __forceinline__ float row_max4(float v) {
  typedef unsigned u2x __attribute__((ext_vector_type(2)));
  const unsigned u = __float_as_uint(v);
  const u2x a = __builtin_amdgcn_permlane32_swap(u, u, false, false);
  const float m = fmaxf(__uint_as_float(a[0]), __uint_as_float(a[1]));
  const unsigned um = __float_as_uint(m);
  const u2x b = __builtin_amdgcn_permlane16_swap(um, um, false, false);
  return fmaxf(__uint_as_float(b[0]), __uint_as_float(b[1]));
}
__device__ __forceinline__ float row_sum4(float v) {
  typedef unsigned u2x __attribute__((ext_vector_type(2)));
  const unsigned u = __float_as_uint(v);
  const u2x a = __builtin_amdgcn_permlane32_swap(u, u, false, false);
  const float m = __uint_as_float(a[0]) + __uint_as_float(a[1]);
  const unsigned um = __float_as_uint(m);
  const u2x b = __builtin_amdgcn_permlane16_swap(um, um, false, false);
  return __uint_as_float(b[0]) + __uint_as_float(b[1]);
}

template <int DH, bool MUBUF = false>
__global__ __launch_bounds__(512) void tok_attn2_kernel(const TokAttnArgs a) {
  constexpr int BK = 32;
  constexpr int CPR = DH / 8;
  constexpr int ROWB = DH * 2;
  constexpr int TILE = BK * ROWB;
  constexpr int SEG = 16;
  constexpr int NP = BK * CPR / 512;
  constexpr int KS = DH / 32;
  constexpr int DBH = DH / 32;
  static_assert(DH == 256 || DH == 512, "wide heads only");
  extern __shared__ __attribute__((aligned(16))) char lds[];
  char* const sKb = lds;
  char* const sVb = lds + 2 * TILE;
  char* const xb = lds + 4 * TILE;
  float* const sbias = reinterpret_cast<float*>(lds + 4 * TILE + 16384);

  const int tid = threadIdx.x;
  const int lane = tid & 63;
  const int w = __builtin_amdgcn_readfirstlane(tid >> 6);
  const int qb = w >> 1, half = w & 1;
  const int l15 = lane & 15, g = lane >> 4;

  int bid;
  {
    const int nwg = gridDim.x, qn = nwg >> 3, rn = nwg & 7;
    const int xcd = blockIdx.x & 7, idx = blockIdx.x >> 3;
    bid = (xcd < rn ? xcd * (qn + 1) : rn * (qn + 1) + (xcd - rn) * qn) + idx;
  }
  const int qblk = bid % a.nqb;
  const int sp = (bid / a.nqb) % a.ns;
  const int bh = bid / (a.nqb * a.ns);
  const int b = bh / a.H, h = bh - b * a.H;
  const int q0 = qblk * 64;
  const int Sq = a.Sq, Skv = a.Skv;
  const int ntile_all = (Skv + BK - 1) / BK;
  const int kt0 = sp * a.tps, kt1 = min(ntile_all, sp * a.tps + a.tps);
  const int kbeg = kt0 * BK;

  const int hkv = h / a.kv_group;
  const bf16_t* kb_ = a.k + (int64_t)b * a.k_bs + hkv * DH;
  const bf16_t* vb_ = a.v + (int64_t)b * a.v_bs + hkv * DH;

  constexpr int RSTEP = 512 / CPR;
  const int row0 = CPR >= 64 ? w : w * 2 + (lane >> 5), cp0 = lane & (CPR - 1);
  uint32_t koff[2], vofs;
#pragma unroll
  for (int j = 0; j < 2; ++j) {
    const int row = row0 + j * RSTEP;
    koff[j] = (uint32_t)row0 * (uint32_t)(a.ldk * 2) + ((cp0 ^ (row & (SEG - 1))) << 4);
  }
  vofs = (uint32_t)row0 * (uint32_t)(a.ldv * 2) + (((cp0 & ~(SEG - 1)) | (((cp0 & (SEG - 1)) - tv_rot<SEG>(row0)) & (SEG - 1))) << 4);
  auto dma_tile = [&](const bf16_t* base, int64_t ld, bool is_k, int kt, char* dst) {
    const char* const tb = reinterpret_cast<const char*>(base) + (int64_t)kt * BK * ld * 2;
    const int ld2 = (int)(ld * 2), tbo = kt * BK * ld2;
    if (kt * BK + BK <= Skv) {
#pragma unroll
      for (int i = 0; i < NP; ++i) {
        if constexpr (MUBUF) {
          lds_dma_mubuf16(base, dst + (i * 512 + w * 64) * 16, (int)(is_k ? koff[i & 1] : vofs), tbo + i * RSTEP * ld2);
        } else {
          const char* const rb = tb + (int64_t)(i * RSTEP) * ld * 2;
          __builtin_amdgcn_global_load_lds((const __attribute__((address_space(1))) void*)(rb + (is_k ? koff[i & 1] : vofs)),
                                           (__attribute__((address_space(3))) void*)(dst + (i * 512 + w * 64) * 16), 16, 0, 0);
        }
      }
    } else {
      const int last = Skv - 1 - kt * BK;
#pragma unroll
      for (int i = 0; i < NP; ++i) {
        const int row = row0 + i * RSTEP;
        if constexpr (MUBUF) {
          const int back = (row - min(row, last)) * ld2;
          lds_dma_mubuf16(base, dst + (i * 512 + w * 64) * 16, (int)(is_k ? koff[i & 1] : vofs) + i * RSTEP * ld2 - back, tbo);
        } else {
          const char* const rb = tb + (int64_t)(i * RSTEP) * ld * 2 - (int64_t)(row - min(row, last)) * ld * 2;
          __builtin_amdgcn_global_load_lds((const __attribute__((address_space(1))) void*)(rb + (is_k ? koff[i & 1] : vofs)),
                                           (__attribute__((address_space(3))) void*)(dst + (i * 512 + w * 64) * 16), 16, 0, 0);
        }
      }
    }
  };
  auto dma_k = [&](int kt, int stage) { dma_tile(kb_, a.ldk, true, kt, sKb + stage * TILE); };
  auto dma_v = [&](int kt, int stage) { dma_tile(vb_, a.ldv, false, kt, sVb + stage * TILE); };

  const bool has_bias = a.rel_bias != nullptr;
  const int tmin = kbeg - (q0 + 63) + a.max_len - 1;
  const int nslot = (kt1 - kt0) * BK + 63;
  float bias_in[2] = {0.f, 0.f};
  if (has_bias) {
#pragma unroll
    for (int r = 0; r < 2; ++r) {
      const int t = tid + 512 * r, row = tmin + t;
      if (t < nslot && row >= 0 && row < 2 * a.max_len - 1) bias_in[r] = bf16_to_f32(a.rel_bias[(int64_t)row * a.H + h]);
    }
  }
  dma_k(kt0, 0);
  const int qrow = q0 + 16 * qb + l15;
  bf16x8 qf[KS];
  {
    const bf16_t* qp = a.q + (int64_t)b * a.q_bs + (int64_t)min(qrow, Sq - 1) * a.ldq + h * DH + g * 8;
#pragma unroll
    for (int ks = 0; ks < KS; ++ks) qf[ks] = *reinterpret_cast<const bf16x8*>(qp + ks * 32);
  }
  dma_v(kt0, 0);
  const bool two = kt0 + 1 < kt1;
  if (two) dma_k(kt0 + 1, 1);
  if (has_bias) {
#pragma unroll
    for (int r = 0; r < 2; ++r)
      if (tid + 512 * r < nslot) sbias[tid + 512 * r] = bias_in[r] * 1.44269504088896340736f;
  }

  const int k_off = (16 * half + l15) * ROWB;
  const int k_swz = l15;
  const int v_row = 4 * g + (l15 >> 2);
  const int v_rot = tv_rot<SEG>(v_row);
  const int v_base_off = v_row * ROWB + (l15 & 1) * 8;
  const int v_cc = (l15 & 3) >> 1;
  uint32_t voff[8];
#pragma unroll
  for (int j = 0; j < 8; ++j) voff[j] = v_base_off + half * (DBH * 32) + (((2 * j + v_cc + v_rot) & (SEG - 1)) << 4);
  const uint32_t v_lds0 = (uint32_t)(uintptr_t)(__attribute__((address_space(3))) char*)sVb;
  const int x_wr = w * 1024 + lane * 16;
  const int x_rd = (2 * qb) * 1024 + lane * 16;

  f32x4 o[DBH];
#pragma unroll
  for (int i = 0; i < DBH; ++i) o[i] = f32x4{0.f, 0.f, 0.f, 0.f};
  float m_run = -INFINITY, l_run = 0.f;
  const float c_scale = a.scale_log2e;
  const int bias_q = q0 + 63 - qrow;

  constexpr int K1 = DH >= 512 ? 4 : 8;
  bf16x8 kf[KS];
  auto scores_begin = [&](int stage) {
    const char* const tK = sKb + stage * TILE + k_off;
#pragma unroll
    for (int ks = 0; ks < K1; ++ks) kf[ks] = *reinterpret_cast<const bf16x8*>(tK + (((ks * 4 + g) ^ k_swz) << 4));
  };
  auto scores_end = [&](int stage, int par) {
    const char* const tK = sKb + stage * TILE + k_off;
    f32x4 acc[4];
#pragma unroll
    for (int i = 0; i < 4; ++i) acc[i] = f32x4{0.f, 0.f, 0.f, 0.f};
    __builtin_amdgcn_sched_barrier(0);
#pragma unroll
    for (int ks = K1; ks < KS; ++ks) kf[ks] = *reinterpret_cast<const bf16x8*>(tK + (((ks * 4 + g) ^ k_swz) << 4));
#pragma unroll
    for (int ks = 0; ks < KS; ++ks) acc[ks & 3] = mfma16(kf[ks], qf[ks], acc[ks & 3]);
#pragma unroll
    for (int ks = 0; ks < KS; ++ks) {
      __builtin_amdgcn_sched_group_barrier(0x008, 1, 0);
      if (ks + K1 < KS) __builtin_amdgcn_sched_group_barrier(0x100, 1, 0);
    }
    __builtin_amdgcn_sched_barrier(0);
    const f32x4 sc = (acc[0] + acc[1]) + (acc[2] + acc[3]);
    *reinterpret_cast<f32x4*>(xb + par * 8192 + x_wr) = sc;
  };

  if (two) asm volatile("s_waitcnt vmcnt(%0)" ::"n"(2 * NP) : "memory");
  else asm volatile("s_waitcnt vmcnt(%0)" ::"n"(NP) : "memory");
  __syncthreads();
  scores_begin(0);
  scores_end(0, 0);
  for (int kt = kt0; kt < kt1; ++kt) {
    const int par = (kt - kt0) & 1;
    const bool more = kt + 1 < kt1;
    asm volatile("s_waitcnt vmcnt(0)" ::: "memory");
    __syncthreads();
    if (more) dma_v(kt + 1, par ^ 1);
    if (kt + 2 < kt1) dma_k(kt + 2, par);
    if (more) scores_begin(par ^ 1);
    constexpr int NX = 8;
    float x[NX];
    {
      const f32x4 s0 = *reinterpret_cast<const f32x4*>(xb + par * 8192 + x_rd);
      const f32x4 s1 = *reinterpret_cast<const f32x4*>(xb + par * 8192 + x_rd + 1024);
      if (has_bias) {
        float bb[NX];
#pragma unroll
        for (int i = 0; i < NX; ++i) bb[i] = sbias[(kt * BK - kbeg) + (i >> 2) * 16 + 4 * g + (i & 3) + bias_q];
#pragma unroll
        for (int i = 0; i < 4; ++i) {
          x[i] = __builtin_fmaf(s0[i], c_scale, bb[i]);
          x[4 + i] = __builtin_fmaf(s1[i], c_scale, bb[4 + i]);
        }
      } else {
#pragma unroll
        for (int i = 0; i < 4; ++i) {
          x[i] = s0[i];
          x[4 + i] = s1[i];
        }
      }
    }
    if (kt == ntile_all - 1 && (Skv & (BK - 1))) {
#pragma unroll
      for (int i = 0; i < NX; ++i)
        if (kt * BK + (i >> 2) * 16 + 4 * g + (i & 3) >= Skv) x[i] = -INFINITY;
    }
    float mt = fmaxf(fmaxf(fmaxf(x[0], x[1]), fmaxf(x[2], x[3])), fmaxf(fmaxf(x[4], x[5]), fmaxf(x[6], x[7])));
    mt = row_max4(mt);
    const float xs = has_bias ? 1.0f : c_scale;
    mt *= xs;
    if (__any(mt > m_run + TOKATTN_RESCALE_THR)) {
      const float m_new = fmaxf(m_run, mt);
      const float alpha = __builtin_amdgcn_exp2f(m_run - m_new);
      m_run = m_new;
      l_run *= alpha;
#pragma unroll
      for (int i = 0; i < DBH; ++i) {
        o[i][0] *= alpha; o[i][1] *= alpha; o[i][2] *= alpha; o[i][3] *= alpha;
      }
    }
#pragma unroll
    for (int i = 0; i < NX; ++i) x[i] = __builtin_amdgcn_exp2f(__builtin_fmaf(x[i], xs, -m_run));
    l_run += ((x[0] + x[1]) + (x[2] + x[3])) + ((x[4] + x[5]) + (x[6] + x[7]));
    union { bf16x8 v; uint32_t u[4]; } pf;
    pf.u[0] = pack2_bf16(x[0], x[1]);
    pf.u[1] = pack2_bf16(x[2], x[3]);
    pf.u[2] = pack2_bf16(x[4], x[5]);
    pf.u[3] = pack2_bf16(x[6], x[7]);
    if (more) scores_end(par ^ 1, par ^ 1);
    {
      const uint32_t tv = v_lds0 + par * TILE;
#define U2_PV_ADDR [a0] "v"(tv + voff[0]), [a1] "v"(tv + voff[1]), [a2] "v"(tv + voff[2]), [a3] "v"(tv + voff[3]), \
                   [a4] "v"(tv + voff[4]), [a5] "v"(tv + voff[5]), [a6] "v"(tv + voff[6]), [a7] "v"(tv + voff[7])
      if constexpr (DBH == 16) {
        asm volatile(TOKATTN_PV_ASM_TEXT_16
                     : [o0] "+v"(o[0]), [o1] "+v"(o[1]), [o2] "+v"(o[2]), [o3] "+v"(o[3]), [o4] "+v"(o[4]), [o5] "+v"(o[5]),
                       [o6] "+v"(o[6]), [o7] "+v"(o[7]), [o8] "+v"(o[8]), [o9] "+v"(o[9]), [o10] "+v"(o[10]), [o11] "+v"(o[11]),
                       [o12] "+v"(o[12]), [o13] "+v"(o[13]), [o14] "+v"(o[14]), [o15] "+v"(o[15])
                     : [pf] "v"(pf.v), U2_PV_ADDR
                     : TOKATTN_PV_ASM_CLOBBERS, "memory");
      } else {
        asm volatile(TOKATTN_PV_ASM_TEXT_8
                     : [o0] "+v"(o[0]), [o1] "+v"(o[1]), [o2] "+v"(o[2]), [o3] "+v"(o[3]), [o4] "+v"(o[4]), [o5] "+v"(o[5]),
                       [o6] "+v"(o[6]), [o7] "+v"(o[7])
                     : [pf] "v"(pf.v), U2_PV_ADDR
                     : TOKATTN_PV_ASM_CLOBBERS, "memory");
      }
#undef U2_PV_ADDR
    }
  }

  const float l_tot = row_sum4(l_run);
  if (qrow >= Sq) return;
  const int d0 = half * (DH / 2) + 4 * g;
  if (a.ns == 1) {
    const float inv = 1.f / l_tot;
    bf16_t* op = a.out + (int64_t)b * a.o_bs + (int64_t)qrow * a.ldo + h * DH + d0;
#pragma unroll
    for (int i = 0; i < DBH; ++i)
      *reinterpret_cast<uint2*>(op + i * 16) =
          uint2{pack2_bf16(o[i][0] * inv, o[i][1] * inv), pack2_bf16(o[i][2] * inv, o[i][3] * inv)};
  } else {
    const int E = a.H * DH;
    float* pp = a.opart + (((int64_t)sp * a.nb + b) * Sq + qrow) * E + h * DH + d0;
#pragma unroll
    for (int i = 0; i < DBH; ++i) *reinterpret_cast<float4*>(pp + i * 16) = float4{o[i][0], o[i][1], o[i][2], o[i][3]};
    if (g == 0 && half == 0) {
      float* mp = a.ml + ((((int64_t)sp * a.nb + b) * a.H + h) * Sq + qrow) * 2;
      mp[0] = m_run;
      mp[1] = l_tot;
    }
  }
}

__global__ __launch_bounds__(256) void tok_attn_combine_kernel(const TokAttnArgs a, int DH) {
  const int E = a.H * DH, e4 = E >> 2;
  const int64_t total = (int64_t)a.nb * a.Sq * e4;
  const int64_t idx = (int64_t)blockIdx.x * 256 + threadIdx.x;
  if (idx >= total) return;
  const int e = (int)(idx % e4) * 4;
  const int64_t bq = idx / e4;
  const int qrow = (int)(bq % a.Sq), b = (int)(bq / a.Sq);
  const int h = e / DH;
  float m = -INFINITY;
  for (int s = 0; s < a.ns; ++s) m = fmaxf(m, a.ml[((((int64_t)s * a.nb + b) * a.H + h) * a.Sq + qrow) * 2]);
  float L = 0.f, acc[4] = {0.f, 0.f, 0.f, 0.f};
  for (int s = 0; s < a.ns; ++s) {
    const float* mp = a.ml + ((((int64_t)s * a.nb + b) * a.H + h) * a.Sq + qrow) * 2;
    const float wgt = __builtin_amdgcn_exp2f(mp[0] - m);
    L += wgt * mp[1];
    const float4 t = *reinterpret_cast<const float4*>(a.opart + (((int64_t)s * a.nb + b) * a.Sq + qrow) * E + e);
    acc[0] += wgt * t.x; acc[1] += wgt * t.y; acc[2] += wgt * t.z; acc[3] += wgt * t.w;
  }
  const float inv = 1.f / L;
  *reinterpret_cast<uint2*>(a.out + (int64_t)b * a.o_bs + (int64_t)qrow * a.ldo + e) =
      uint2{pack2_bf16(acc[0] * inv, acc[1] * inv), pack2_bf16(acc[2] * inv, acc[3] * inv)};
}

template <int NS>
__global__ __launch_bounds__(256) void tok_attn_combine_ns_kernel(const TokAttnArgs a, int DH) {
  const int E = a.H * DH, e4 = E >> 2;
  const int64_t total = (int64_t)a.nb * a.Sq * e4;
  const int64_t idx = (int64_t)blockIdx.x * 256 + threadIdx.x;
  if (idx >= total) return;
  const int e = (int)(idx % e4) * 4;
  const int64_t bq = idx / e4;
  const int qrow = (int)(bq % a.Sq), b = (int)(bq / a.Sq);
  const int h = e / DH;
  float2 ml[NS];
  float4 t[NS];
#pragma unroll
  for (int s = 0; s < NS; ++s) {
    ml[s] = *reinterpret_cast<const float2*>(a.ml + ((((int64_t)s * a.nb + b) * a.H + h) * a.Sq + qrow) * 2);
    t[s] = *reinterpret_cast<const float4*>(a.opart + (((int64_t)s * a.nb + b) * a.Sq + qrow) * E + e);
  }
  float m = -INFINITY;
#pragma unroll
  for (int s = 0; s < NS; ++s) m = fmaxf(m, ml[s].x);
  float L = 0.f, acc[4] = {0.f, 0.f, 0.f, 0.f};
#pragma unroll
  for (int s = 0; s < NS; ++s) {
    const float wgt = __builtin_amdgcn_exp2f(ml[s].x - m);
    L += wgt * ml[s].y;
    acc[0] += wgt * t[s].x; acc[1] += wgt * t[s].y; acc[2] += wgt * t[s].z; acc[3] += wgt * t[s].w;
  }
  const float inv = 1.f / L;
  *reinterpret_cast<uint2*>(a.out + (int64_t)b * a.o_bs + (int64_t)qrow * a.ldo + e) =
      uint2{pack2_bf16(acc[0] * inv, acc[1] * inv), pack2_bf16(acc[2] * inv, acc[3] * inv)};
}

static inline int tok_attn_bk(int d) { return d <= 128 ? 64 : 32; }

static int tok_attn_pick_splits(int nb, int H, int Sq, int Skv, int d, size_t ws_bytes) {
  const int64_t base = (int64_t)nb * H * cdiv(Sq, 64);
  const int ntile = (int)cdiv(Skv, tok_attn_bk(d));
  if (base >= 192 || ntile < 4) return 1;
  int ns = (int)std::min<int64_t>(cdiv(256, base), ntile / 2);
  const size_t per = (size_t)nb * Sq * ((size_t)H * d * 4 + (size_t)H * 8);
  if (per == 0 || ws_bytes / per < 2) return 1;
  ns = (int)std::min<size_t>((size_t)ns, ws_bytes / per);
  return std::max(ns, 1);
}

size_t tok_attention_workspace_bytes(int nb, int H, int Sq, int Skv, int d) {
  const int64_t base = (int64_t)nb * H * cdiv(Sq, 64);
  const int ntile = (int)cdiv(Skv, tok_attn_bk(d));
  if (base >= 192 || ntile < 4) return 0;
  const int ns = (int)std::min<int64_t>(cdiv(256, base), ntile / 2);
  return (size_t)ns * nb * Sq * ((size_t)H * d * 4 + (size_t)H * 8);
}

bool tok_attention_supported(const bf16_t* q, const bf16_t* k, const bf16_t* v, const bf16_t* out, int Sq, int Skv, int d,
                             int64_t ldq, int64_t ldk, int64_t ldv, int64_t ldo, int64_t q_bs, int64_t k_bs, int64_t v_bs,
                             int64_t o_bs, const bf16_t* rel_bias, int max_len) {
  if (d != 64 && d != 96 && d != 128 && d != 256 && d != 512) return false;
  if ((ldq | ldk | ldv | q_bs | k_bs | v_bs) & 7) return false;
  if ((ldo | o_bs) & 3) return false;
  if ((((uintptr_t)q | (uintptr_t)k | (uintptr_t)v) & 15) || ((uintptr_t)out & 7)) return false;
  if (rel_bias && (Sq > max_len || Skv > max_len || (int)cdiv(Skv, 64) * 64 + 63 > TOKATTN_BIAS_SLOTS)) return false;
  return true;
}

int tok_attention(const bf16_t* q, const bf16_t* k, const bf16_t* v, bf16_t* out, int nb, int Sq, int Skv, int H, int d,
                  int64_t ldq, int64_t ldk, int64_t ldv, int64_t ldo, int64_t q_bs, int64_t k_bs, int64_t v_bs, int64_t o_bs,
                  float scale, const bf16_t* rel_bias, int max_len, int force_splits, void* ws, size_t ws_bytes,
                  hipStream_t stream) {
  return attention_ex(q, k, v, out, nb, Sq, Skv, H, H, d, ldq, ldk, ldv, ldo, q_bs, k_bs, v_bs, o_bs, scale, rel_bias, max_len, 0,
                      force_splits, ws, ws_bytes, stream);
}

int attention_ex(const bf16_t* q, const bf16_t* k, const bf16_t* v, bf16_t* out, int nb, int Sq, int Skv, int H, int Hkv, int d,
                 int64_t ldq, int64_t ldk, int64_t ldv, int64_t ldo, int64_t q_bs, int64_t k_bs, int64_t v_bs, int64_t o_bs,
                 float scale, const bf16_t* rel_bias, int max_len, int causal, int force_splits, void* ws, size_t ws_bytes,
                 hipStream_t stream) {
  if (!q || !k || !v || !out || nb <= 0 || Sq <= 0 || Skv <= 0 || H <= 0 || Hkv <= 0 || H % Hkv) return U2_ERR_ARG;
  if (causal && (Skv < Sq || rel_bias)) return U2_ERR_ARG;
  if (!tok_attention_supported(q, k, v, out, Sq, Skv, d, ldq, ldk, ldv, ldo, q_bs, k_bs, v_bs, o_bs, rel_bias, max_len))
    return U2_ERR_ARG;
  TokAttnArgs a;
  a.q = q; a.k = k; a.v = v; a.out = out;
  a.ldq = ldq; a.ldk = ldk; a.ldv = ldv; a.ldo = ldo; a.q_bs = q_bs; a.k_bs = k_bs; a.v_bs = v_bs; a.o_bs = o_bs;
  a.nb = nb; a.H = H; a.Sq = Sq; a.Skv = Skv; a.nqb = (int)cdiv(Sq, 64);
  a.scale_log2e = scale * 1.44269504088896340736f;
  a.rel_bias = rel_bias; a.max_len = max_len;
  const int ntile = (int)cdiv(Skv, tok_attn_bk(d));
  a.kv_group = H / Hkv;
  a.causal = causal ? 1 : 0;
  a.kv_len = nullptr; a.lse = nullptr; a.lse_ld = 0;
  int ns = force_splits > 0 ? std::min(force_splits, ntile) : tok_attn_pick_splits(nb, H, Sq, Skv, d, ws ? ws_bytes : 0);
  if (causal) ns = 1;
  const size_t per = (size_t)nb * Sq * ((size_t)H * d * 4 + (size_t)H * 8);
  if (ns > 1 && (!ws || ws_bytes < (size_t)ns * per || ((uintptr_t)ws & 15))) {
    if (force_splits > 0) return U2_ERR_WORKSPACE;
    ns = 1;
  }
  a.tps = (int)cdiv(ntile, ns);
  a.ns = (int)cdiv(ntile, a.tps);
  a.opart = nullptr; a.ml = nullptr;
  if (a.ns > 1) {
    a.opart = reinterpret_cast<float*>(ws);
    a.ml = a.opart + (size_t)a.ns * nb * Sq * H * d;
  }
  const int64_t grid = (int64_t)nb * H * a.nqb * a.ns;
  if (grid > 0x7fffffff) return U2_ERR_ARG;
  ProfScope ps(PROF_TOKATTN, (causal ? 2.0 : 4.0) * nb * H * (double)Sq * Skv * d, stream,
               2.0 * nb * d * (2.0 * Sq * H + 2.0 * Skv * Hkv));
#define U2_TA(D_)                                                                                                      \
  do {                                                                                                                 \
    constexpr size_t smem_ = 4 * ((D_) <= 128 ? 64 : 32) * (D_) * 2 + TOKATTN_BIAS_SLOTS * 4;                          \
    hipLaunchKernelGGL((tok_attn_kernel<D_>), dim3((unsigned)grid), dim3(256), smem_, stream, a);                      \
  } while (0)
#define U2_TA2(D_)                                                                                                     \
  do {                                                                                                                 \
    constexpr size_t smem_ = 4 * 32 * (D_) * 2 + 16384 + TOKATTN_BIAS_SLOTS * 4;                                       \
    if (mubuf) hipLaunchKernelGGL((tok_attn2_kernel<D_, true>), dim3((unsigned)grid), dim3(512), smem_, stream, a);    \
    else hipLaunchKernelGGL((tok_attn2_kernel<D_, false>), dim3((unsigned)grid), dim3(512), smem_, stream, a);         \
  } while (0)
  const bool wide = d >= 256 && !causal && opts().tok_wide;
  const bool mubuf = opts().tok_wide == 2 && (int64_t)Skv * ldk < (1ll << 29) && (int64_t)Skv * ldv < (1ll << 29);
  if (d == 512) { if (wide) U2_TA2(512); else U2_TA(512); }
  else if (d == 256) { if (wide) U2_TA2(256); else U2_TA(256); }
  else if (d == 128) U2_TA(128);
  else if (d == 96) U2_TA(96);
  else U2_TA(64);
#undef U2_TA
#undef U2_TA2
  if (a.ns > 1) {
    const int64_t total = (int64_t)nb * Sq * (H * d / 4);
    const dim3 cg((unsigned)cdiv(total, 256));
#define U2_CMB(NS_) case NS_: hipLaunchKernelGGL(tok_attn_combine_ns_kernel<NS_>, cg, dim3(256), 0, stream, a, d); break
    switch (a.ns <= 8 ? a.ns : 0) {
      U2_CMB(2); U2_CMB(3); U2_CMB(4); U2_CMB(5); U2_CMB(6); U2_CMB(7); U2_CMB(8);
      default: hipLaunchKernelGGL(tok_attn_combine_kernel, cg, dim3(256), 0, stream, a, d);
    }
#undef U2_CMB

  }
  return launch_status();
}

int attention_gqa_ex(const bf16_t* q, const bf16_t* k, const bf16_t* v, bf16_t* out, int nb, int Sq, int Skv, int H, int Hkv,
                     int d, int64_t ldq, int64_t ldk, int64_t ldv, int64_t ldo, int64_t q_bs, int64_t k_bs, int64_t v_bs,
                     int64_t o_bs, float scale, int causal, const int* kv_len, float* lse, int64_t lse_ld,
                     hipStream_t stream) {
  if (!kv_len && !lse)
    return attention_ex(q, k, v, out, nb, Sq, Skv, H, Hkv, d, ldq, ldk, ldv, ldo, q_bs, k_bs, v_bs, o_bs, scale, nullptr, 0,
                        causal, 1, nullptr, 0, stream);
  if (!q || !k || !v || !out || nb <= 0 || Sq <= 0 || Skv <= 0 || H <= 0 || Hkv <= 0 || H % Hkv) return U2_ERR_ARG;
  if ((causal && Skv < Sq) || ((uintptr_t)kv_len & 3) || ((uintptr_t)lse & 3) || (lse && lse_ld < Sq)) return U2_ERR_ARG;
  if (!tok_attention_supported(q, k, v, out, Sq, Skv, d, ldq, ldk, ldv, ldo, q_bs, k_bs, v_bs, o_bs, nullptr, 0))
    return U2_ERR_ARG;
  TokAttnArgs a;
  a.q = q; a.k = k; a.v = v; a.out = out;
  a.ldq = ldq; a.ldk = ldk; a.ldv = ldv; a.ldo = ldo; a.q_bs = q_bs; a.k_bs = k_bs; a.v_bs = v_bs; a.o_bs = o_bs;
  a.nb = nb; a.H = H; a.Sq = Sq; a.Skv = Skv; a.nqb = (int)cdiv(Sq, 64);
  a.scale_log2e = scale * 1.44269504088896340736f;
  a.rel_bias = nullptr; a.max_len = 0;
  a.kv_group = H / Hkv;
  a.causal = causal ? 1 : 0;
  a.kv_len = kv_len; a.lse = lse; a.lse_ld = lse_ld;
  a.ns = 1;
  a.tps = (int)cdiv(Skv, tok_attn_bk(d));
  a.opart = nullptr; a.ml = nullptr;
  const int64_t grid = (int64_t)nb * H * a.nqb;
  if (grid > 0x7fffffff) return U2_ERR_ARG;
  ProfScope ps(PROF_TOKATTN, (causal ? 2.0 : 4.0) * nb * H * (double)Sq * Skv * d, stream,
               2.0 * nb * d * (2.0 * Sq * H + 2.0 * Skv * Hkv));
#define U2_TAX(D_)                                                                                                     \
  do {                                                                                                                 \
    constexpr size_t smem_ = 4 * ((D_) <= 128 ? 64 : 32) * (D_) * 2 + TOKATTN_BIAS_SLOTS * 4;                          \
    hipLaunchKernelGGL((tok_attn_kernel<D_, true>), dim3((unsigned)grid), dim3(256), smem_, stream, a);                \
  } while (0)
  if (d == 512) U2_TAX(512);
  else if (d == 256) U2_TAX(256);
  else if (d == 128) U2_TAX(128);
  else if (d == 96) U2_TAX(96);
  else U2_TAX(64);
#undef U2_TAX
  return launch_status();
}

}
```

### u2tokenizer_amd/tokenizer.py

```python
from __future__ import annotations

import ctypes as C

import torch
import torch.nn as nn

from . import _lib, ops

_ATTN_TYPES = {"rma": 0, "rope": 1}


def _init_attn(m):
    for lin in (m.wq, m.wk, m.wv, m.dense):
        nn.init.xavier_uniform_(lin.weight)
        if lin.bias is not None:
            nn.init.zeros_(lin.bias)


class RelativeMultiheadAttention(nn.Module):

    def __init__(self, d_model, num_heads, max_seq_len=512):
        super().__init__()
        assert d_model % num_heads == 0
        self.num_heads, self.d_model, self.depth, self.max_seq_len = num_heads, d_model, d_model // num_heads, max_seq_len
        self.wq = nn.Linear(d_model, d_model)
        self.wk = nn.Linear(d_model, d_model)
        self.wv = nn.Linear(d_model, d_model)
        self.dense = nn.Linear(d_model, d_model)
        self.relative_bias = nn.Parameter(torch.zeros(2 * max_seq_len - 1, num_heads))
        self._reset_parameters()

    def _reset_parameters(self):
        _init_attn(self)
        nn.init.zeros_(self.relative_bias)

    init_weights = _reset_parameters


class RotaryMultiheadAttention(nn.Module):

    def __init__(self, d_model, num_heads, max_seq_len=512):
        super().__init__()
        assert d_model % num_heads == 0, "d_model must be divisible by num_heads"
        self.num_heads, self.d_model, self.head_dim, self.max_seq_len = num_heads, d_model, d_model // num_heads, max_seq_len
        self.wq = nn.Linear(d_model, d_model)
        self.wk = nn.Linear(d_model, d_model)
        self.wv = nn.Linear(d_model, d_model)
        self.dense = nn.Linear(d_model, d_model)
        self._reset_parameters()

    def _reset_parameters(self):
        _init_attn(self)


class MultiHeadCrossAttention(nn.Module):

    def __init__(self, d_model, num_heads):
        super().__init__()
        assert d_model % num_heads == 0
        self.num_heads, self.d_model, self.depth = num_heads, d_model, d_model // num_heads
        self.wq = nn.Linear(d_model, d_model)
        self.wk = nn.Linear(d_model, d_model)
        self.wv = nn.Linear(d_model, d_model)
        self.dense = nn.Linear(d_model, d_model)
        _init_attn(self)


def _self_attention(embed_size, num_heads, attn_type):
    if attn_type == "rma":
        return RelativeMultiheadAttention(embed_size, num_heads)
    if attn_type == "rope":
        return RotaryMultiheadAttention(embed_size, num_heads)
    return nn.MultiheadAttention(embed_size, num_heads)


class SpatioTemporalAttentionLayer(nn.Module):
    def __init__(self, embed_size, num_heads, attn_type="rma"):
        super().__init__()
        self.spatial_attention = _self_attention(embed_size, num_heads, attn_type)
        self.temporal_attention = _self_attention(embed_size, num_heads, attn_type)


class SpatioTemporalSignificanceScoring(nn.Module):
    def __init__(self, embed_size, num_heads, num_layers, attn_type="rma"):
        super().__init__()
        self.layers = nn.ModuleList(
            [SpatioTemporalAttentionLayer(embed_size, num_heads, attn_type) for _ in range(num_layers)])


class TokenSelection(nn.Module):
    def __init__(self, embed_size, top_k):
        super().__init__()
        self.score_net = nn.Linear(embed_size, 1)
        self.top_k = top_k
        self.score_net.bias.data.zero_()


class DifferentiableTokenSelection(nn.Module):
    def __init__(self, embed_size, top_k, tau=1.0):
        super().__init__()
        self.score_net = nn.Linear(embed_size, top_k)
        self.top_k = top_k
        self.tau = tau


class DynamicMultiScalePooling(nn.Module):
    def __init__(self, embed_size, scales=(1, 2, 4)):
        super().__init__()
        if list(scales) != [1, 2, 4]:
            raise ValueError("the HIP pooling kernel implements the reference's scales [1, 2, 4] (svr.py:120,177)")
        self.scales = list(scales)
        self.gate_fc = nn.Linear(embed_size, 1)


class SpatioTemporalVisualTokenRefinerModel(nn.Module):
    def __init__(self, embed_size, num_heads, num_layers, top_k, use_multi_scale, attn_type="rma",
                 enable_diffts=False, enable_dmtp=False):
        super().__init__()
        self.attention_network = SpatioTemporalSignificanceScoring(embed_size, num_heads, num_layers, attn_type)
        if enable_diffts:
            self.token_selection = DifferentiableTokenSelection(embed_size, top_k)
        else:
            self.token_selection = TokenSelection(embed_size, top_k)
        if enable_dmtp:
            self.dynamic_pool = DynamicMultiScalePooling(embed_size)
        self.enable_dmtp = enable_dmtp
        self.use_multi_scale = use_multi_scale


class TextConditionTokenAttMap(nn.Module):
    def __init__(self, d_model, num_heads, attn_type="rma"):
        super().__init__()
        self.visual_cross_attention = MultiHeadCrossAttention(d_model, num_heads)
        self.text_cross_attention = MultiHeadCrossAttention(d_model, num_heads)
        self.dropout_cross = nn.Identity()
        self.norm_cross_v = nn.LayerNorm(d_model)
        self.norm_cross_t = nn.LayerNorm(d_model)
        self.self_attention = _self_attention(d_model, num_heads, attn_type)
        self.dropout_self = nn.Identity()
        self.norm_self = nn.LayerNorm(d_model)


class LinearAggregation(nn.Module):
    def __init__(self, d_model, num_heads):
        super().__init__()
        self.linear_aggregator = MultiHeadCrossAttention(d_model, num_heads)


class TextConditionTokenAggregatorModel(nn.Module):
    def __init__(self, d_model, num_layers, num_heads, attn_type="rma"):
        super().__init__()
        self.layers_vt = nn.ModuleList([TextConditionTokenAttMap(d_model, num_heads, attn_type)
                                        for _ in range(num_layers)])
        self.layer_linagg = LinearAggregation(d_model, num_heads)


def _pack_qkv(m) -> None:
    if isinstance(m, nn.MultiheadAttention):
        return
    _pack_qkv_linear(m)


def _pack_qkv_linear(m) -> None:
    ws, bs = [m.wq.weight, m.wk.weight, m.wv.weight], [m.wq.bias, m.wk.bias, m.wv.bias]
    E = ws[0].shape[0]
    step_w, step_b = ws[0].numel() * ws[0].element_size(), bs[0].numel() * bs[0].element_size()
    if all(w.is_contiguous() for w in ws) and all(ws[i + 1].data_ptr() == ws[i].data_ptr() + step_w for i in (0, 1)) \
            and all(bs[i + 1].data_ptr() == bs[i].data_ptr() + step_b for i in (0, 1)):
        return
    W = torch.cat([w.data for w in ws], 0).contiguous()
    Bv = torch.cat([b.data for b in bs], 0).contiguous()
    for i in range(3):
        ws[i].data = W[i * E:(i + 1) * E]
        bs[i].data = Bv[i * E:(i + 1) * E]


def _att_ptrs(m, value_side: bool = True):
    if not value_side:
        return [m.wq.weight, m.wq.bias, m.wk.weight, m.wk.bias, None, None, None, None, None]
    if isinstance(m, nn.MultiheadAttention):
        E = m.embed_dim
        W, b = m.in_proj_weight, m.in_proj_bias
        return [W[:E], b[:E], W[E:2 * E], b[E:2 * E], W[2 * E:], b[2 * E:], m.out_proj.weight, m.out_proj.bias, None]
    return [m.wq.weight, m.wq.bias, m.wk.weight, m.wk.bias, m.wv.weight, m.wv.bias, m.dense.weight, m.dense.bias,
            getattr(m, "relative_bias", None)]


def _unshare_packed(module, state_dict, prefix, local_metadata):
    for k, v in list(state_dict.items()):
        if k.startswith(prefix) and torch.is_tensor(v) and \
                v.untyped_storage().nbytes() != v.numel() * v.element_size():
            state_dict[k] = v.detach().clone() if not v.requires_grad else v.clone().detach()
    return state_dict


class u2Tokenizer(nn.Module):

    def __init__(self, embed_size, num_heads, num_layers, top_k, use_multi_scale, num_3d_query_token, hidden_size,
                 attn_type="rma", enable_diffts=False, enable_dmtp=False):
        super().__init__()
        if embed_size != hidden_size:
            raise ValueError("embed_size must equal hidden_size (builder.py:5,11 pass config.hidden_size for both)")
        self.svt_module = SpatioTemporalVisualTokenRefinerModel(
            embed_size=embed_size, num_heads=num_heads, num_layers=num_layers, top_k=top_k,
            use_multi_scale=use_multi_scale, attn_type=attn_type, enable_diffts=enable_diffts,
            enable_dmtp=enable_dmtp)
        self.tta_module = TextConditionTokenAggregatorModel(d_model=embed_size, num_layers=num_layers,
                                                            num_heads=num_heads, attn_type=attn_type)
        self.query_tokens = nn.Parameter(torch.zeros(1, num_3d_query_token, hidden_size))
        self.query_tokens.data.normal_(mean=0.0, std=0.02)
        self.embed_size, self.num_heads, self.num_layers, self.top_k = embed_size, num_heads, num_layers, top_k
        self.use_multi_scale, self.num_query, self.attn_type = bool(use_multi_scale), num_3d_query_token, attn_type
        self.enable_diffts, self.enable_dmtp = bool(enable_diffts), bool(enable_dmtp)
        self._ws = ops._Workspace()
        self._packed_key = None
        self._dead_offloaded = False
        self._register_state_dict_hook(_unshare_packed)
        self.last_topk_indices = None
        self.capture_svr_tokens = False
        self.last_svr_tokens = None

    def _weights(self):
        w = [self.query_tokens]
        for layer in self.svt_module.attention_network.layers:
            w += _att_ptrs(layer.spatial_attention) + _att_ptrs(layer.temporal_attention)
        sn = self.svt_module.token_selection.score_net
        w += [sn.weight, sn.bias]
        if self.enable_dmtp:
            w += [self.svt_module.dynamic_pool.gate_fc.weight, self.svt_module.dynamic_pool.gate_fc.bias]
        else:
            w += [None, None]
        for layer in self.tta_module.layers_vt:
            w += _att_ptrs(layer.self_attention) + _att_ptrs(layer.visual_cross_attention) \
                + _att_ptrs(layer.text_cross_attention)
            w += [layer.norm_self.weight, layer.norm_self.bias, layer.norm_cross_v.weight, layer.norm_cross_v.bias,
                  layer.norm_cross_t.weight, layer.norm_cross_t.bias]
        w += _att_ptrs(self.tta_module.layer_linagg.linear_aggregator, value_side=False)
        return w

    def pack_weights(self) -> None:
        key = (self.query_tokens.data_ptr(), self.query_tokens.dtype)
        if self._packed_key == key:
            return
        with torch.no_grad():
            for layer in self.svt_module.attention_network.layers:
                _pack_qkv(layer.spatial_attention)
                _pack_qkv(layer.temporal_attention)
            for layer in self.tta_module.layers_vt:
                for m in (layer.self_attention, layer.visual_cross_attention, layer.text_cross_attention):
                    _pack_qkv(m)
        if self.query_tokens.is_cuda:
            torch.cuda.synchronize(self.query_tokens.device)
        self._packed_key = key

    def _apply(self, fn, *args, **kwargs):
        r = super()._apply(fn, *args, **kwargs)
        self._packed_key = None
        if self.query_tokens.is_cuda:
            self.pack_weights()
            if self._dead_offloaded:
                self.offload_dead_parameters()
        return r

    def dead_parameters(self):
        la = self.tta_module.layer_linagg.linear_aggregator
        return [la.wv.weight, la.wv.bias, la.dense.weight, la.dense.bias]

    def offload_dead_parameters(self) -> int:
        freed = 0
        for p in self.dead_parameters():
            if p.is_cuda:
                freed += p.numel() * p.element_size()
                p.data = p.data.to("cpu")
            p.requires_grad_(False)
        self._dead_offloaded = True
        return freed

    def _check_envelope(self, B, T, N, E, Lt):
        H = self.num_heads
        if E % H or (E // H) % 8:
            raise RuntimeError(f"head dim {E}/{H} must be a multiple of 8 (16-byte fragment loads)")
        if max(N, T, self.num_query) > 512:
            raise RuntimeError(f"sequence lengths N={N}, T={T}, queries={self.num_query} must be <= max_seq_len = 512 "
                               "(relative-bias table / RoPE cache of the reference, rma.py:6,64-68, rope.py:19)")
        if not self.enable_diffts:
            if self.top_k > T * N:
                raise RuntimeError(f"top_k={self.top_k} > T*N={T * N}: torch.topk would raise in the reference (svr.py:82)")
            if T * N > 8192:
                raise RuntimeError(f"hard top-k sorts T*N={T * N} scores in one workgroup's LDS: limit 8192")

    def forward_with_taps(self, v_token, t_token, svr_in=None, visual_in=None, tta_in=None):
        with ops.on_device(v_token, elem=self.query_tokens.dtype):
            return self._forward_with_taps(v_token, t_token, svr_in, visual_in, tta_in)

    def _forward_with_taps(self, v_token, t_token, svr_in, visual_in, tta_in):
        h = _lib.load_library()
        self.pack_weights()
        v_token = ops._need(v_token, ops.ELEM, "v_token").contiguous()
        t_token = ops._need(t_token, ops.ELEM, "t_token").contiguous()
        (B, T, N, E) = v_token.size()
        self._check_envelope(B, T, N, E, t_token.shape[1])
        L, Q, dev = self.num_layers, self.num_query, v_token.device
        Lv = self.top_k + (self.top_k // 2 + self.top_k // 4 if self.use_multi_scale else 0)
        cfg = self._config(B, T, N, E, t_token.shape[1])
        table = ops.weight_table(self._weights())
        nbytes = h.u2tok_tokenizer_workspace_bytes(C.byref(cfg))
        keep = []

        def ptr_array(tensors, shape):
            arr = (C.c_void_p * L)()
            for i in range(L):
                t = tensors[i] if tensors is not None and i < len(tensors) else None
                if t is not None:
                    t = ops._need(t, ops.ELEM, "tap").contiguous()
                    assert tuple(t.shape) == shape, (tuple(t.shape), shape)
                    keep.append(t)
                    arr[i] = t.data_ptr()
            return arr

        svr_out = [torch.empty((B, T, N, E), dtype=ops.elem_dtype(), device=dev) for _ in range(L)]
        tta_out = [torch.empty((B, Q, E), dtype=ops.elem_dtype(), device=dev) for _ in range(L)]
        visual_out = torch.empty((B, Lv, E), dtype=ops.elem_dtype(), device=dev)
        if visual_in is not None:
            visual_in = ops._need(visual_in, ops.ELEM, "visual_in").contiguous()
            assert tuple(visual_in.shape) == (B, Lv, E)
        taps = _lib.TokTaps(svr_in=ptr_array(svr_in, (B, T, N, E)), svr_out=ptr_array(svr_out, (B, T, N, E)),
                            visual_in=None if visual_in is None else visual_in.data_ptr(), visual_out=visual_out.data_ptr(),
                            tta_in=ptr_array(tta_in, (B, Q, E)), tta_out=ptr_array(tta_out, (B, Q, E)))
        with ops.on_device(v_token) as (h, stream):
            ws = self._ws.get(nbytes, dev)
            out = torch.empty((B, Q, E), dtype=ops.elem_dtype(), device=dev)
            idx = None if self.enable_diffts else torch.empty((B, self.top_k), dtype=torch.int64, device=dev)
            _lib.check(h.u2tok_tokenizer_forward_taps(C.byref(cfg), table, v_token.data_ptr(), t_token.data_ptr(),
                                                      out.data_ptr(), None if idx is None else idx.data_ptr(),
                                                      C.byref(taps), ws.data_ptr(), ws.numel(), stream),
                       "u2tok_tokenizer_forward_taps")
        self.last_topk_indices = idx
        return out, {"svr_out": svr_out, "visual_out": visual_out, "tta_out": tta_out}

    def _config(self, B, T, N, E, Lt):
        return _lib.TokConfig(B=B, T=T, N=N, E=E, Lt=Lt, num_heads=self.num_heads,
                              num_layers=self.num_layers, top_k=self.top_k, num_query=self.num_query,
                              use_multi_scale=int(self.use_multi_scale), attn_type=_ATTN_TYPES.get(self.attn_type, 2),
                              enable_diffts=int(self.enable_diffts), enable_dmtp=int(self.enable_dmtp),
                              max_seq_len=512, diffts_tau=float(getattr(self.svt_module.token_selection, "tau", 1.0)),
                              ln_eps=1e-5)

    def forward(self, v_token, t_token):
        with ops.on_device(v_token, elem=self.query_tokens.dtype):
            return self._forward(v_token, t_token)

    def _forward(self, v_token, t_token):
        if torch.is_grad_enabled() and (v_token.requires_grad or t_token.requires_grad
                                        or any(p.requires_grad for p in self.parameters())):
            from . import autograd as AG
            ops.training_needs_bf16(self.query_tokens.dtype, "u2Tokenizer")
            ops._need(v_token, ops.ELEM, "v_token"), ops._need(t_token, ops.ELEM, "t_token")
            (B, T, N, E) = v_token.size()
            self._check_envelope(B, T, N, E, t_token.shape[1])
            with ops.on_device(v_token):
                return AG.tokenizer_forward(self, v_token, t_token)
        h = _lib.load_library()
        if self.query_tokens.is_cuda:
            self.pack_weights()
        v_token = ops._need(v_token, ops.ELEM, "v_token").contiguous()
        t_token = ops._need(t_token, ops.ELEM, "t_token").contiguous()
        (B, T, N, E) = v_token.size()
        if E != self.embed_size or t_token.shape[0] != B or t_token.shape[2] != E:
            raise RuntimeError(f"shape mismatch: v_token {tuple(v_token.shape)}, t_token {tuple(t_token.shape)}")
        self._check_envelope(B, T, N, E, t_token.shape[1])
        cfg = self._config(B, T, N, E, t_token.shape[1])
        table = ops.weight_table(self._weights())
        nbytes = h.u2tok_tokenizer_workspace_bytes(C.byref(cfg))
        if nbytes == 0:
            raise RuntimeError("u2tok_tokenizer_workspace_bytes rejected the configuration "
                               f"(B={B}, T={T}, N={N}, E={E}, heads={self.num_heads}, top_k={self.top_k})")
        idx = svr = None
        with ops.on_device(v_token) as (h, stream):
            ws = self._ws.get(nbytes, v_token.device)
            out = torch.empty((B, self.num_query, E), dtype=ops.elem_dtype(), device=v_token.device)
            if not self.enable_diffts:
                idx = torch.empty((B, self.top_k), dtype=torch.int64, device=v_token.device)
            if self.capture_svr_tokens:
                svr = torch.empty((B, T * N, E), dtype=ops.elem_dtype(), device=v_token.device)
            _lib.check(h.u2tok_tokenizer_forward(C.byref(cfg), table, v_token.data_ptr(), t_token.data_ptr(),
                                                 out.data_ptr(), None if idx is None else idx.data_ptr(),
                                                 None if svr is None else svr.data_ptr(), ws.data_ptr(), ws.numel(),
                                                 stream), "u2tok_tokenizer_forward")
        self.last_topk_indices = idx
        self.last_svr_tokens = svr
        return out
```

Before: 125.9 volumes/s.

## Merge all TTA cross-attention K/V projections into two wide GEMMs

Weight packing now lays out every layer's visual-cross K/V weights, plus the linear-aggregator K, in one contiguous block, and the text-cross K/V weights in another. This lets the tokenizer compute all layers' K/V projections with two wide GEMMs up front instead of per-layer GEMMs or side-stream overlap, and attention reads them with a larger leading dimension. Separately, an opt-in path (off by default) uses per-unit atomic tickets so the last split-K block merges partial attention results inside the same launch, dropping the combine kernel. The merged path gives up side-stream overlap and needs a larger single workspace, and the ticket path relies on cross-block memory fences.

Result: no change. 126.2 volumes/s (median of 6 runs) (+0.2%).

```diff
diff --git a/u2tokenizer_amd/checkpoint.py b/u2tokenizer_amd/checkpoint.py
--- a/u2tokenizer_amd/checkpoint.py
+++ b/u2tokenizer_amd/checkpoint.py
@@ -63,11 +63,12 @@
 
 
 def packing_report(model: torch.nn.Module) -> Dict[str, int]:
+    from .tokenizer import MultiHeadCrossAttention
     n = packed = 0
     for m in model.modules():
         if all(hasattr(m, a) for a in ("wq", "wk", "wv")) and hasattr(m.wq, "weight"):
             n += 1
-            w = [m.wq.weight, m.wk.weight, m.wv.weight]
+            w = [m.wk.weight, m.wv.weight] if isinstance(m, MultiHeadCrossAttention) else [m.wq.weight, m.wk.weight, m.wv.weight]
             step = w[0].numel() * w[0].element_size()
-            packed += int(all(w[i + 1].data_ptr() == w[i].data_ptr() + step for i in (0, 1)))
+            packed += int(all(b.data_ptr() == a.data_ptr() + step for a, b in zip(w, w[1:])))
     return {"attention_modules": n, "qkv_packed": packed}
diff --git a/u2tokenizer_amd/csrc/capi.hip b/u2tokenizer_amd/csrc/capi.hip
--- a/u2tokenizer_amd/csrc/capi.hip
+++ b/u2tokenizer_amd/csrc/capi.hip
@@ -59,6 +59,7 @@
       {"vit_vt_epilogue", &Options::vit_vt_epilogue, 0, 1},
       {"tok_flash", &Options::tok_flash, 0, 1},
       {"tok_wide", &Options::tok_wide, 0, 2},
+      {"tta_kv_merged", &Options::tta_kv_merged, 0, 1},  {"tok_merge_in_launch", &Options::tok_merge_in_launch, 0, 1},
   };
   if (!strcmp(name, "gemm_tile")) {
     if (value != 0 && value != 64 && value != 128) return U2_ERR_ARG;
diff --git a/u2tokenizer_amd/csrc/ctx.h b/u2tokenizer_amd/csrc/ctx.h
--- a/u2tokenizer_amd/csrc/ctx.h
+++ b/u2tokenizer_amd/csrc/ctx.h
@@ -24,6 +24,8 @@
   int tok_flash = 1;
   int tok_wide = 2;
   int tta_overlap = 1;
+  int tta_kv_merged = 1;
+  int tok_merge_in_launch = 0;
   int profile = 0;
 };
 
@@ -40,6 +42,11 @@
   size_t bytes;
 };
 
+struct Tickets {
+  hipStream_t st;
+  unsigned* p;
+};
+
 struct ProfRec {
   hipEvent_t a, b;
   int cat;
@@ -51,6 +58,8 @@
   std::mutex mu;
   std::vector<SideStream*> sides;
   std::vector<Scratch> scratch;
+  std::vector<Tickets> tickets;
+  static constexpr int kTickets = 4096;
   std::vector<ProfRec> recs;
   std::vector<hipEvent_t> ev_pool;
   size_t ev_used = 0;
@@ -58,6 +67,7 @@
   SideStream* side_for(hipStream_t owner);
   void set_scratch(hipStream_t st, void* p, size_t bytes);
   Scratch scratch_of(hipStream_t st);
+  unsigned* tickets_for(hipStream_t st);
   void release();
   ~Context() { release(); }
 };
diff --git a/u2tokenizer_amd/csrc/ctx.hip b/u2tokenizer_amd/csrc/ctx.hip
--- a/u2tokenizer_amd/csrc/ctx.hip
+++ b/u2tokenizer_amd/csrc/ctx.hip
@@ -43,8 +43,24 @@
   return {st, nullptr, 0};
 }
 
+unsigned* Context::tickets_for(hipStream_t st) {
+  std::lock_guard<std::mutex> lk(mu);
+  for (auto& t : tickets)
+    if (t.st == st) return t.p;
+  unsigned* p = nullptr;
+  if (hipMalloc(&p, kTickets * sizeof(unsigned)) != hipSuccess || hipMemset(p, 0, kTickets * sizeof(unsigned)) != hipSuccess) {
+    (void)hipGetLastError();
+    if (p) (void)hipFree(p);
+    return nullptr;
+  }
+  tickets.push_back({st, p});
+  return p;
+}
+
 void Context::release() {
   std::lock_guard<std::mutex> lk(mu);
+  for (auto& t : tickets) (void)hipFree(t.p);
+  tickets.clear();
   for (SideStream* s : sides) {
     (void)hipStreamDestroy(s->s);
     (void)hipEventDestroy(s->fork);
diff --git a/u2tokenizer_amd/csrc/pipeline.hip b/u2tokenizer_amd/csrc/pipeline.hip
--- a/u2tokenizer_amd/csrc/pipeline.hip
+++ b/u2tokenizer_amd/csrc/pipeline.hip
@@ -303,6 +303,12 @@
 inline bool qkv_packed(const Att& a, int E) {
   return a.wq && a.bq && a.wk == a.wq + (size_t)E * E && a.bk == a.bq + E && kv_packed(a, E);
 }
+inline bool kv_merged(const Att* a, int n, const Att* tail, int E) {
+  if (n <= 0 || !kv_packed(a[0], E)) return false;
+  for (int l = 1; l < n; ++l)
+    if (!kv_packed(a[l], E) || a[l].wk != a[0].wk + (size_t)2 * l * E * E || a[l].bk != a[0].bk + (size_t)2 * l * E) return false;
+  return !tail || (tail->wk && tail->bk && tail->wk == a[0].wk + (size_t)2 * n * E * E && tail->bk == a[0].bk + (size_t)2 * n * E);
+}
 int qkv_proj(const bf16_t* x, const Att& a, bf16_t* out, int64_t rows, int E, bool dry, hipStream_t st) {
   if (!dry && qkv_packed(a, E)) {
     U2_RUN(linear(x, E, a.wq, a.bq, out, 3 * E, rows, E, 3 * E, 0, nullptr, 0, st));
@@ -487,18 +493,44 @@
   bf16_t* qproj = ar.get<bf16_t>((size_t)qrows * 3 * E);
   bf16_t* qctx = ar.get<bf16_t>((size_t)qrows * E);
   bf16_t* qo = ar.get<bf16_t>((size_t)qrows * E);
-  SideStream* side = (!dry && opts().tta_overlap && L > 0 && L <= 7) ? cx.side_for(st) : nullptr;
+  Att va_all[8], ta_all[8];
+  bool mergeable = L > 0 && L <= 8 && (dry || opts().tta_kv_merged != 0);
+  if (mergeable && !dry) {
+    for (int l = 0; l < L; ++l) {
+      va_all[l] = att_at(i_tta + 33 * l + 9);
+      ta_all[l] = att_at(i_tta + 33 * l + 18);
+    }
+    const Att la = att_at(i_lin);
+    mergeable = kv_merged(va_all, L, &la, E) && kv_merged(ta_all, L, nullptr, E);
+  }
+  const bool merged = mergeable && !dry;
+  SideStream* side = (!dry && !merged && opts().tta_overlap && L > 0 && L <= 7) ? cx.side_for(st) : nullptr;
   const bool overlap = dry ? (L > 0 && L <= 7) : side != nullptr;
+  const int64_t ldV = (int64_t)(2 * L + 1) * E, ldT = (int64_t)2 * L * E;
   const int Lmax = Lv > c.Lt ? Lv : c.Lt;
-  bf16_t* kv_inline = overlap ? nullptr : ar.get<bf16_t>((size_t)B * Lmax * 2 * E);
+  const size_t kv_mark = ar.off;
+  size_t kv_end_merged = kv_mark;
+  bf16_t *kvV = nullptr, *kvT = nullptr;
+  if (mergeable) {
+    kvV = ar.get<bf16_t>((size_t)B * Lv * ldV);
+    kvT = ar.get<bf16_t>((size_t)B * c.Lt * ldT);
+    kv_end_merged = ar.off;
+  }
+  bf16_t* kv_inline = nullptr;
   bf16_t* kv_v[8] = {};
   bf16_t* kv_t[8] = {};
-  if (overlap)
-    for (int l = 0; l < L; ++l) {
-      kv_v[l] = ar.get<bf16_t>((size_t)B * Lv * 2 * E);
-      kv_t[l] = ar.get<bf16_t>((size_t)B * c.Lt * 2 * E);
-    }
-  bf16_t* k_lin = ar.get<bf16_t>((size_t)B * Lv * E);
+  bf16_t* k_lin = nullptr;
+  if (!merged) {
+    ar.off = kv_mark;
+    kv_inline = overlap ? nullptr : ar.get<bf16_t>((size_t)B * Lmax * 2 * E);
+    if (overlap)
+      for (int l = 0; l < L; ++l) {
+        kv_v[l] = ar.get<bf16_t>((size_t)B * Lv * 2 * E);
+        kv_t[l] = ar.get<bf16_t>((size_t)B * c.Lt * 2 * E);
+      }
+    k_lin = ar.get<bf16_t>((size_t)B * Lv * E);
+    if (ar.off < kv_end_merged) ar.off = kv_end_merged;
+  }
   U2_CHECK_WS(ar);
   auto kv_proj = [&](const Att& a, const bf16_t* src, int Ls, bf16_t* kv, hipStream_t s_) -> int {
     if (!dry && kv_packed(a, E)) {
@@ -512,6 +544,12 @@
   if (overlap && !dry) {
     if (hipEventRecord(side->fork, st) != hipSuccess || hipStreamWaitEvent(side->s, side->fork, 0) != hipSuccess)
       return U2_ERR_LAUNCH;
+  }
+  if (merged) {
+    ScratchScope no_split(cx, st, nullptr, 0, true);
+    U2_RUN(linear(V, E, va_all[0].wk, va_all[0].bk, kvV, ldV, (int64_t)B * Lv, E, (int)ldV, 0, nullptr, 0, st));
+    U2_RUN(linear(t_token, E, ta_all[0].wk, ta_all[0].bk, kvT, ldT, (int64_t)B * c.Lt, E, (int)ldT, 0, nullptr, 0, st));
+  } else if (overlap && !dry) {
     for (int l = 0; l < L; ++l) {
       const int base = i_tta + 33 * l;
       Att va = att_at(base + 9), ta = att_at(base + 18);
@@ -526,16 +564,16 @@
   }
   U2_RUN(fill_rows(wp(0), qa, B, (int64_t)Q * E, (int64_t)Q * E, st));
   bf16_t* qcur = qa;
-  auto cross = [&](const Att& a, const bf16_t* src, int Ls, const bf16_t* qin, bf16_t* dst, bf16_t* kv,
+  auto cross = [&](const Att& a, const bf16_t* src, int Ls, const bf16_t* qin, bf16_t* dst, bf16_t* kv, int64_t ldkv,
                    int kv_ready) -> int {
     U2_RUN(linear(qin, E, a.wq, a.bq, qproj, E, qrows, E, E, 0, nullptr, 0, st));
-    if (kv_ready < 0) {
+    if (kv_ready == -1) {
       const int e = kv_proj(a, src, Ls, kv, st);
       if (e != U2_OK) return e;
-    } else if (!dry) {
+    } else if (!dry && kv_ready >= 0) {
       if (hipStreamWaitEvent(st, side->done[kv_ready], 0) != hipSuccess) return U2_ERR_LAUNCH;
     }
-    AttnCore ac{qproj, kv, kv + E, E, 2 * E, 2 * E, (int64_t)Q * E, (int64_t)Ls * 2 * E, (int64_t)Ls * 2 * E,
+    AttnCore ac{qproj, kv, kv + E, E, ldkv, ldkv, (int64_t)Q * E, (int64_t)Ls * ldkv, (int64_t)Ls * ldkv,
                 qctx, E, (int64_t)Q * E, B, Q, Ls, H, d, scale, nullptr, 0};
     const int e = attention_core(ar, ac, dry, st);
     if (e != U2_OK) return e;
@@ -571,9 +609,17 @@
     }
     U2_RUN(linear(qctx, E, sa.wd, sa.bd, qo, E, qrows, E, E, 0, nullptr, 0, st));
     U2_RUN(layernorm_bf16(qcur, qo, ns_w, ns_b, s1, 1, (int)qrows, E, 0, E, 0, E, 0, E, c.ln_eps, st));
-    { const int e = cross(va, V, Lv, s1, qo, overlap ? kv_v[l] : kv_inline, overlap ? 2 * l : -1); if (e != U2_OK) return e; }
+    {
+      const int e = merged ? cross(va, V, Lv, s1, qo, kvV + (int64_t)2 * l * E, ldV, -2)
+                           : cross(va, V, Lv, s1, qo, overlap ? kv_v[l] : kv_inline, 2 * E, overlap ? 2 * l : -1);
+      if (e != U2_OK) return e;
+    }
     U2_RUN(layernorm_bf16(s1, qo, nv_w, nv_b, s2, 1, (int)qrows, E, 0, E, 0, E, 0, E, c.ln_eps, st));
-    { const int e = cross(ta, t_token, c.Lt, s2, qo, overlap ? kv_t[l] : kv_inline, overlap ? 2 * l + 1 : -1); if (e != U2_OK) return e; }
+    {
+      const int e = merged ? cross(ta, t_token, c.Lt, s2, qo, kvT + (int64_t)2 * l * E, ldT, -2)
+                           : cross(ta, t_token, c.Lt, s2, qo, overlap ? kv_t[l] : kv_inline, 2 * E, overlap ? 2 * l + 1 : -1);
+      if (e != U2_OK) return e;
+    }
     U2_RUN(layernorm_bf16(s2, qo, nt_w, nt_b, s1, 1, (int)qrows, E, 0, E, 0, E, 0, E, c.ln_eps, st));
     qcur = s1;
     if (taps && !dry && taps->tta_out && taps->tta_out[l] &&
@@ -583,12 +629,15 @@
   {
     const Att la = att_at(i_lin);
     U2_RUN(linear(qcur, E, la.wq, la.bq, qproj, E, qrows, E, E, 0, nullptr, 0, st));
-    if (!overlap) {
+    if (merged) {
+      k_lin = kvV + (int64_t)2 * L * E;
+    } else if (!overlap) {
       U2_RUN(linear(V, E, la.wk, la.bk, k_lin, E, (int64_t)B * Lv, E, E, 0, nullptr, 0, st));
     } else if (!dry) {
       if (hipStreamWaitEvent(st, side->done[2 * L], 0) != hipSuccess) return U2_ERR_LAUNCH;
     }
-    AttnCore ac{qproj, k_lin, V, E, E, E, (int64_t)Q * E, (int64_t)Lv * E, (int64_t)Lv * E,
+    const int64_t ldkl = merged ? ldV : E;
+    AttnCore ac{qproj, k_lin, V, E, ldkl, E, (int64_t)Q * E, (int64_t)Lv * ldkl, (int64_t)Lv * E,
                 out, E, (int64_t)Q * E, B, Q, Lv, H, d, scale, nullptr, 0};
     const int e = attention_core(ar, ac, dry, st);
     if (e != U2_OK) return e;
diff --git a/u2tokenizer_amd/csrc/tokattn.hip b/u2tokenizer_amd/csrc/tokattn.hip
--- a/u2tokenizer_amd/csrc/tokattn.hip
+++ b/u2tokenizer_amd/csrc/tokattn.hip
@@ -18,6 +18,7 @@
   int max_len;
   float* opart;
   float* ml;
+  unsigned* tickets;
   int kv_group;
   int causal;
   const int* kv_len;
@@ -37,6 +38,81 @@
 __device__ __forceinline__ int t96_pos(int row, int L) { return L ^ ((row >> 1) & 2); }
 
 typedef short ta_v4s_t __attribute__((ext_vector_type(4)));
+
+template <int NS>
+__device__ __forceinline__ void tok_attn_merge4(const TokAttnArgs& a, int DH, int b, int h, int qrow, int e) {
+  const int E = a.H * DH;
+  float L = 0.f, acc[4] = {0.f, 0.f, 0.f, 0.f};
+  if constexpr (NS > 0) {
+    float2 ml[NS];
+    float4 t[NS];
+#pragma unroll
+    for (int s = 0; s < NS; ++s) {
+      ml[s] = *reinterpret_cast<const float2*>(a.ml + ((((int64_t)s * a.nb + b) * a.H + h) * a.Sq + qrow) * 2);
+      t[s] = *reinterpret_cast<const float4*>(a.opart + (((int64_t)s * a.nb + b) * a.Sq + qrow) * E + e);
+    }
+    float m = -INFINITY;
+#pragma unroll
+    for (int s = 0; s < NS; ++s) m = fmaxf(m, ml[s].x);
+#pragma unroll
+    for (int s = 0; s < NS; ++s) {
+      const float wgt = __builtin_amdgcn_exp2f(ml[s].x - m);
+      L += wgt * ml[s].y;
+      acc[0] += wgt * t[s].x; acc[1] += wgt * t[s].y; acc[2] += wgt * t[s].z; acc[3] += wgt * t[s].w;
+    }
+  } else {
+    float m = -INFINITY;
+    for (int s = 0; s < a.ns; ++s) m = fmaxf(m, a.ml[((((int64_t)s * a.nb + b) * a.H + h) * a.Sq + qrow) * 2]);
+    for (int s = 0; s < a.ns; ++s) {
+      const float* mp = a.ml + ((((int64_t)s * a.nb + b) * a.H + h) * a.Sq + qrow) * 2;
+      const float wgt = __builtin_amdgcn_exp2f(mp[0] - m);
+      L += wgt * mp[1];
+      const float4 t = *reinterpret_cast<const float4*>(a.opart + (((int64_t)s * a.nb + b) * a.Sq + qrow) * E + e);
+      acc[0] += wgt * t.x; acc[1] += wgt * t.y; acc[2] += wgt * t.z; acc[3] += wgt * t.w;
+    }
+  }
+  const float inv = 1.f / L;
+  *reinterpret_cast<uint2*>(a.out + (int64_t)b * a.o_bs + (int64_t)qrow * a.ldo + e) =
+      uint2{pack2_bf16(acc[0] * inv, acc[1] * inv), pack2_bf16(acc[2] * inv, acc[3] * inv)};
+}
+
+template <int NS, int NT>
+__device__ __forceinline__ void tok_attn_unit_rows(const TokAttnArgs& a, int DH, int b, int h, int q0, int tid) {
+  const int c4 = DH >> 2, rows = min(64, a.Sq - q0);
+  for (int i = tid; i < rows * c4; i += NT) tok_attn_merge4<NS>(a, DH, b, h, q0 + i / c4, h * DH + (i % c4) * 4);
+}
+template <int NT>
+__device__ __forceinline__ void tok_attn_merge_in_launch(const TokAttnArgs& a, int DH, int b, int h, int qblk, int tid,
+                                                         volatile int* flag) {
+  asm volatile("s_waitcnt vmcnt(0)" ::: "memory");
+  __syncthreads();
+  const int unit = (b * a.H + h) * a.nqb + qblk;
+  if (tid == 0) {
+    __builtin_amdgcn_fence(__ATOMIC_RELEASE, "agent");
+    asm volatile("s_waitcnt vmcnt(0)" ::: "memory");
+    const unsigned t = __hip_atomic_fetch_add(a.tickets + unit, 1u, __ATOMIC_RELAXED, __HIP_MEMORY_SCOPE_AGENT);
+    const int last = t == (unsigned)(a.ns - 1);
+    if (last) {
+      __builtin_amdgcn_fence(__ATOMIC_ACQUIRE, "agent");
+      asm volatile("s_waitcnt vmcnt(0)" ::: "memory");
+    }
+    *flag = last;
+  }
+  __syncthreads();
+  if (!*flag) return;
+  const int q0 = qblk * 64;
+  switch (a.ns) {
+    case 2: tok_attn_unit_rows<2, NT>(a, DH, b, h, q0, tid); break;
+    case 3: tok_attn_unit_rows<3, NT>(a, DH, b, h, q0, tid); break;
+    case 4: tok_attn_unit_rows<4, NT>(a, DH, b, h, q0, tid); break;
+    case 5: tok_attn_unit_rows<5, NT>(a, DH, b, h, q0, tid); break;
+    case 6: tok_attn_unit_rows<6, NT>(a, DH, b, h, q0, tid); break;
+    case 7: tok_attn_unit_rows<7, NT>(a, DH, b, h, q0, tid); break;
+    case 8: tok_attn_unit_rows<8, NT>(a, DH, b, h, q0, tid); break;
+    default: tok_attn_unit_rows<0, NT>(a, DH, b, h, q0, tid);
+  }
+  if (tid == 0) __hip_atomic_store(a.tickets + unit, 0u, __ATOMIC_RELAXED, __HIP_MEMORY_SCOPE_AGENT);
+}
 
 template <int DH, bool EX = false>
 __global__ __launch_bounds__(256, DH >= 512 ? 1 : 2) void tok_attn_kernel(const TokAttnArgs a) {
@@ -274,11 +350,12 @@
 
   float l_tot = l_run + __shfl_xor(l_run, 16, 64);
   l_tot += __shfl_xor(l_tot, 32, 64);
-  if (qrow >= Sq) return;
+  const bool live = qrow < Sq;
   if constexpr (EX) {
-    if (a.lse && g == 0) a.lse[((int64_t)b * a.H + h) * a.lse_ld + qrow] = m_run + __builtin_log2f(l_tot);
+    if (live && a.lse && g == 0) a.lse[((int64_t)b * a.H + h) * a.lse_ld + qrow] = m_run + __builtin_log2f(l_tot);
   }
   if (a.ns == 1) {
+    if (!live) return;
     const float inv = 1.f / l_tot;
     bf16_t* op = a.out + (int64_t)b * a.o_bs + (int64_t)qrow * a.ldo + h * DH + 4 * g;
 #pragma unroll
@@ -286,14 +363,19 @@
       *reinterpret_cast<uint2*>(op + db * 16) =
           uint2{pack2_bf16(o[db][0] * inv, o[db][1] * inv), pack2_bf16(o[db][2] * inv, o[db][3] * inv)};
   } else {
-    const int E = a.H * DH;
-    float* pp = a.opart + (((int64_t)sp * a.nb + b) * Sq + qrow) * E + h * DH + 4 * g;
-#pragma unroll
-    for (int db = 0; db < DB; ++db) *reinterpret_cast<float4*>(pp + db * 16) = float4{o[db][0], o[db][1], o[db][2], o[db][3]};
-    if (g == 0) {
-      float* mp = a.ml + ((((int64_t)sp * a.nb + b) * a.H + h) * Sq + qrow) * 2;
-      mp[0] = m_run;
-      mp[1] = l_tot;
+    if (live) {
+      const int E = a.H * DH;
+      float* pp = a.opart + (((int64_t)sp * a.nb + b) * Sq + qrow) * E + h * DH + 4 * g;
+#pragma unroll
+      for (int db = 0; db < DB; ++db) *reinterpret_cast<float4*>(pp + db * 16) = float4{o[db][0], o[db][1], o[db][2], o[db][3]};
+      if (g == 0) {
+        float* mp = a.ml + ((((int64_t)sp * a.nb + b) * a.H + h) * Sq + qrow) * 2;
+        mp[0] = m_run;
+        mp[1] = l_tot;
+      }
+    }
+    if constexpr (!EX) {
+      if (a.tickets) tok_attn_merge_in_launch<256>(a, DH, b, h, qblk, tid, reinterpret_cast<volatile int*>(lds));
     }
   }
 }
@@ -563,9 +645,10 @@
   }
 
   const float l_tot = row_sum4(l_run);
-  if (qrow >= Sq) return;
+  const bool live = qrow < Sq;
   const int d0 = half * (DH / 2) + 4 * g;
   if (a.ns == 1) {
+    if (!live) return;
     const float inv = 1.f / l_tot;
     bf16_t* op = a.out + (int64_t)b * a.o_bs + (int64_t)qrow * a.ldo + h * DH + d0;
 #pragma unroll
@@ -573,40 +656,19 @@
       *reinterpret_cast<uint2*>(op + i * 16) =
           uint2{pack2_bf16(o[i][0] * inv, o[i][1] * inv), pack2_bf16(o[i][2] * inv, o[i][3] * inv)};
   } else {
-    const int E = a.H * DH;
-    float* pp = a.opart + (((int64_t)sp * a.nb + b) * Sq + qrow) * E + h * DH + d0;
-#pragma unroll
-    for (int i = 0; i < DBH; ++i) *reinterpret_cast<float4*>(pp + i * 16) = float4{o[i][0], o[i][1], o[i][2], o[i][3]};
-    if (g == 0 && half == 0) {
-      float* mp = a.ml + ((((int64_t)sp * a.nb + b) * a.H + h) * Sq + qrow) * 2;
-      mp[0] = m_run;
-      mp[1] = l_tot;
-    }
-  }
-}
-
-__global__ __launch_bounds__(256) void tok_attn_combine_kernel(const TokAttnArgs a, int DH) {
-  const int E = a.H * DH, e4 = E >> 2;
-  const int64_t total = (int64_t)a.nb * a.Sq * e4;
-  const int64_t idx = (int64_t)blockIdx.x * 256 + threadIdx.x;
-  if (idx >= total) return;
-  const int e = (int)(idx % e4) * 4;
-  const int64_t bq = idx / e4;
-  const int qrow = (int)(bq % a.Sq), b = (int)(bq / a.Sq);
-  const int h = e / DH;
-  float m = -INFINITY;
-  for (int s = 0; s < a.ns; ++s) m = fmaxf(m, a.ml[((((int64_t)s * a.nb + b) * a.H + h) * a.Sq + qrow) * 2]);
-  float L = 0.f, acc[4] = {0.f, 0.f, 0.f, 0.f};
-  for (int s = 0; s < a.ns; ++s) {
-    const float* mp = a.ml + ((((int64_t)s * a.nb + b) * a.H + h) * a.Sq + qrow) * 2;
-    const float wgt = __builtin_amdgcn_exp2f(mp[0] - m);
-    L += wgt * mp[1];
-    const float4 t = *reinterpret_cast<const float4*>(a.opart + (((int64_t)s * a.nb + b) * a.Sq + qrow) * E + e);
-    acc[0] += wgt * t.x; acc[1] += wgt * t.y; acc[2] += wgt * t.z; acc[3] += wgt * t.w;
-  }
-  const float inv = 1.f / L;
-  *reinterpret_cast<uint2*>(a.out + (int64_t)b * a.o_bs + (int64_t)qrow * a.ldo + e) =
-      uint2{pack2_bf16(acc[0] * inv, acc[1] * inv), pack2_bf16(acc[2] * inv, acc[3] * inv)};
+    if (live) {
+      const int E = a.H * DH;
+      float* pp = a.opart + (((int64_t)sp * a.nb + b) * Sq + qrow) * E + h * DH + d0;
+#pragma unroll
+      for (int i = 0; i < DBH; ++i) *reinterpret_cast<float4*>(pp + i * 16) = float4{o[i][0], o[i][1], o[i][2], o[i][3]};
+      if (g == 0 && half == 0) {
+        float* mp = a.ml + ((((int64_t)sp * a.nb + b) * a.H + h) * Sq + qrow) * 2;
+        mp[0] = m_run;
+        mp[1] = l_tot;
+      }
+    }
+    if (a.tickets) tok_attn_merge_in_launch<512>(a, DH, b, h, qblk, tid, reinterpret_cast<volatile int*>(lds));
+  }
 }
 
 template <int NS>
@@ -617,28 +679,7 @@
   if (idx >= total) return;
   const int e = (int)(idx % e4) * 4;
   const int64_t bq = idx / e4;
-  const int qrow = (int)(bq % a.Sq), b = (int)(bq / a.Sq);
-  const int h = e / DH;
-  float2 ml[NS];
-  float4 t[NS];
-#pragma unroll
-  for (int s = 0; s < NS; ++s) {
-    ml[s] = *reinterpret_cast<const float2*>(a.ml + ((((int64_t)s * a.nb + b) * a.H + h) * a.Sq + qrow) * 2);
-    t[s] = *reinterpret_cast<const float4*>(a.opart + (((int64_t)s * a.nb + b) * a.Sq + qrow) * E + e);
-  }
-  float m = -INFINITY;
-#pragma unroll
-  for (int s = 0; s < NS; ++s) m = fmaxf(m, ml[s].x);
-  float L = 0.f, acc[4] = {0.f, 0.f, 0.f, 0.f};
-#pragma unroll
-  for (int s = 0; s < NS; ++s) {
-    const float wgt = __builtin_amdgcn_exp2f(ml[s].x - m);
-    L += wgt * ml[s].y;
-    acc[0] += wgt * t[s].x; acc[1] += wgt * t[s].y; acc[2] += wgt * t[s].z; acc[3] += wgt * t[s].w;
-  }
-  const float inv = 1.f / L;
-  *reinterpret_cast<uint2*>(a.out + (int64_t)b * a.o_bs + (int64_t)qrow * a.ldo + e) =
-      uint2{pack2_bf16(acc[0] * inv, acc[1] * inv), pack2_bf16(acc[2] * inv, acc[3] * inv)};
+  tok_attn_merge4<NS>(a, DH, (int)(bq / a.Sq), e / DH, (int)(bq % a.Sq), e);
 }
 
 static inline int tok_attn_bk(int d) { return d <= 128 ? 64 : 32; }
@@ -708,10 +749,11 @@
   }
   a.tps = (int)cdiv(ntile, ns);
   a.ns = (int)cdiv(ntile, a.tps);
-  a.opart = nullptr; a.ml = nullptr;
+  a.opart = nullptr; a.ml = nullptr; a.tickets = nullptr;
   if (a.ns > 1) {
     a.opart = reinterpret_cast<float*>(ws);
     a.ml = a.opart + (size_t)a.ns * nb * Sq * H * d;
+    if (opts().tok_merge_in_launch && (int64_t)nb * H * a.nqb <= Context::kTickets) a.tickets = ctx().tickets_for(stream);
   }
   const int64_t grid = (int64_t)nb * H * a.nqb * a.ns;
   if (grid > 0x7fffffff) return U2_ERR_ARG;
@@ -737,13 +779,13 @@
   else U2_TA(64);
 #undef U2_TA
 #undef U2_TA2
-  if (a.ns > 1) {
+  if (a.ns > 1 && !a.tickets) {
     const int64_t total = (int64_t)nb * Sq * (H * d / 4);
     const dim3 cg((unsigned)cdiv(total, 256));
 #define U2_CMB(NS_) case NS_: hipLaunchKernelGGL(tok_attn_combine_ns_kernel<NS_>, cg, dim3(256), 0, stream, a, d); break
     switch (a.ns <= 8 ? a.ns : 0) {
       U2_CMB(2); U2_CMB(3); U2_CMB(4); U2_CMB(5); U2_CMB(6); U2_CMB(7); U2_CMB(8);
-      default: hipLaunchKernelGGL(tok_attn_combine_kernel, cg, dim3(256), 0, stream, a, d);
+      default: hipLaunchKernelGGL(tok_attn_combine_ns_kernel<0>, cg, dim3(256), 0, stream, a, d);
     }
 #undef U2_CMB
 
@@ -773,7 +815,7 @@
   a.kv_len = kv_len; a.lse = lse; a.lse_ld = lse_ld;
   a.ns = 1;
   a.tps = (int)cdiv(Skv, tok_attn_bk(d));
-  a.opart = nullptr; a.ml = nullptr;
+  a.opart = nullptr; a.ml = nullptr; a.tickets = nullptr;
   const int64_t grid = (int64_t)nb * H * a.nqb;
   if (grid > 0x7fffffff) return U2_ERR_ARG;
   ProfScope ps(PROF_TOKATTN, (causal ? 2.0 : 4.0) * nb * H * (double)Sq * Skv * d, stream,
diff --git a/u2tokenizer_amd/tokenizer.py b/u2tokenizer_amd/tokenizer.py
--- a/u2tokenizer_amd/tokenizer.py
+++ b/u2tokenizer_amd/tokenizer.py
@@ -161,18 +161,40 @@
     _pack_qkv_linear(m)
 
 
-def _pack_qkv_linear(m) -> None:
-    ws, bs = [m.wq.weight, m.wk.weight, m.wv.weight], [m.wq.bias, m.wk.bias, m.wv.bias]
-    E = ws[0].shape[0]
-    step_w, step_b = ws[0].numel() * ws[0].element_size(), bs[0].numel() * bs[0].element_size()
-    if all(w.is_contiguous() for w in ws) and all(ws[i + 1].data_ptr() == ws[i].data_ptr() + step_w for i in (0, 1)) \
-            and all(bs[i + 1].data_ptr() == bs[i].data_ptr() + step_b for i in (0, 1)):
+def _pack_rows(linears) -> None:
+    ws, bs = [l.weight for l in linears], [l.bias for l in linears]
+
+    def adjacent(ts):
+        return all(t.is_contiguous() for t in ts) and all(
+            b.data_ptr() == a.data_ptr() + a.numel() * a.element_size() for a, b in zip(ts, ts[1:]))
+
+    if adjacent(ws) and adjacent(bs):
         return
     W = torch.cat([w.data for w in ws], 0).contiguous()
     Bv = torch.cat([b.data for b in bs], 0).contiguous()
-    for i in range(3):
-        ws[i].data = W[i * E:(i + 1) * E]
-        bs[i].data = Bv[i * E:(i + 1) * E]
+    r0 = b0 = 0
+    for w, b in zip(ws, bs):
+        w.data, b.data = W[r0:r0 + w.shape[0]], Bv[b0:b0 + b.shape[0]]
+        r0, b0 = r0 + w.shape[0], b0 + b.shape[0]
+
+
+def _pack_qkv_linear(m) -> None:
+    _pack_rows([m.wq, m.wk, m.wv])
+
+
+def _pack_kv_sources(tta) -> None:
+    layers = list(tta.layers_vt)
+    if not layers:
+        return
+    vis = [lin for layer in layers for lin in (layer.visual_cross_attention.wk, layer.visual_cross_attention.wv)]
+    txt = [lin for layer in layers for lin in (layer.text_cross_attention.wk, layer.text_cross_attention.wv)]
+    _pack_rows(vis + [tta.layer_linagg.linear_aggregator.wk])
+    _pack_rows(txt)
+    for layer in layers:
+        for m in (layer.visual_cross_attention, layer.text_cross_attention):
+            for t in (m.wq.weight, m.wq.bias):
+                if t.untyped_storage().nbytes() != t.numel() * t.element_size():
+                    t.data = t.data.clone()
 
 
 def _att_ptrs(m, value_side: bool = True):
@@ -247,8 +269,8 @@
                 _pack_qkv(layer.spatial_attention)
                 _pack_qkv(layer.temporal_attention)
             for layer in self.tta_module.layers_vt:
-                for m in (layer.self_attention, layer.visual_cross_attention, layer.text_cross_attention):
-                    _pack_qkv(m)
+                _pack_qkv(layer.self_attention)
+            _pack_kv_sources(self.tta_module)
         if self.query_tokens.is_cuda:
             torch.cuda.synchronize(self.query_tokens.device)
         self._packed_key = key
```
